# scale-lab/MTLoRA

Measured on AMD Instinct MI355X. Metric: images/sec (train step) Swin-T/448 r=64 4-task, higher is better.
Workload: dtype bf16; 1 GPU; BASELINE configs[1]: Swin-T 448, 4 tasks (semseg,normals,sal,human_parts), r_shared=64 r_task=4 scale4; train step (fwd+loss+bwd+clip+AdamW), dropout .05, drop_path .2; per_gpu_batch=32, global_batch=32, img_size=448, parallelism=dp1, trainable_params=8344634, allreduce_bytes=0

## Files before the change

include/mtlora_hip.h:

```cpp
#ifndef MTLORA_HIP_H
#define MTLORA_HIP_H

#include <stdint.h>

#ifdef __cplusplus
extern "C" {
#endif

#define MTLORA_ABI_VERSION 12
#define MTLORA_MAX_TASKS 8

typedef enum mtlora_dtype {
    MTLORA_F32 = 0,
    MTLORA_BF16 = 1,
    MTLORA_F16 = 2,
    MTLORA_U8 = 3
} mtlora_dtype;

typedef enum mtlora_status {
    MTLORA_OK = 0,
    MTLORA_ERR_DTYPE = -1,
    MTLORA_ERR_SHAPE = -2,
    MTLORA_ERR_ALIGN = -3,
    MTLORA_ERR_NULL = -4,
    MTLORA_ERR_WORKSPACE = -5,
    MTLORA_ERR_HIP = -6,
    MTLORA_ERR_UNSUPPORTED = -7
} mtlora_status;

int mtlora_version(void);
const char* mtlora_error_string(int status);

int mtlora_roll_and_window_partition_forward(const void* image, void* windows, int64_t B, int64_t H, int64_t W,
                                             int64_t C, int shift_size, int window_size, int dtype, void* stream);
int mtlora_roll_and_window_partition_backward(const void* grad_windows, void* grad_image, int64_t B, int64_t H,
                                              int64_t W, int64_t C, int shift_size, int window_size, int dtype,
                                              void* stream);
int mtlora_window_merge_and_roll_forward(const void* windows, void* image, int64_t B, int64_t H, int64_t W,
                                         int64_t C, int shift_size, int window_size, int dtype, void* stream);
int mtlora_window_merge_and_roll_backward(const void* grad_image, void* grad_windows, int64_t B, int64_t H,
                                          int64_t W, int64_t C, int shift_size, int window_size, int dtype,
                                          void* stream);

typedef struct mtlora_linear_desc {
    int64_t M, K, N;
    int32_t dtype;
    int32_t mode;
    int32_t T;
    int32_t r_s;
    int32_t r_t[MTLORA_MAX_TASKS];
    float scale_s;
    float scale_t[MTLORA_MAX_TASKS];
    int32_t has_x_tasks;
    float dropout_p;
    uint64_t seed;
    const uint64_t* seed_offset;
    int32_t bwd_phase;
    int32_t sel_stream;
    int32_t sel_dense;
    int32_t sel_tn;
    int32_t sel_projk;
    int32_t max_cu;
    const void* packed;
    int32_t hid;
    int32_t hid_pad_;
    const void* hid_ptr;
} mtlora_linear_desc;

#define MTLORA_HID_FWD_BASE 1
#define MTLORA_HID_P_GIVEN 2
#define MTLORA_HID_Q_GIVEN 4

int64_t mtlora_linear_ctx_bytes(const mtlora_linear_desc* d);

int64_t mtlora_linear_packed_bytes(const mtlora_linear_desc* d);
int mtlora_linear_pack(const mtlora_linear_desc* d, const float* A_s, const float* B_s, const float* const* A_t,
                       const float* const* B_t, void* packed, int64_t packed_bytes, void* stream);
int64_t mtlora_linear_pack_entry_bytes(void);
int mtlora_linear_pack_entry(const mtlora_linear_desc* d, const float* A_s, const float* B_s, const float* const* A_t,
                             const float* const* B_t, void* packed, int64_t packed_bytes, void* entry_host);
int mtlora_linear_pack_table(const void* table_dev, int n_entries, int dtype, void* stream);
int64_t mtlora_linear_bwd_scratch_bytes(const mtlora_linear_desc* d);

int mtlora_linear_fwd(const mtlora_linear_desc* d, const void* x, const void* const* x_t, const void* W,
                      const float* bias, const float* A_s, const float* B_s, const float* const* A_t,
                      const float* const* B_t, void* y_s, void* const* y_t, void* ctx, int64_t ctx_bytes,
                      void* stream);

int mtlora_linear_bwd(const mtlora_linear_desc* d, const void* x, const void* const* x_t, const void* Wt,
                      const void* dy_s, const void* const* dy_t, const void* ctx, int64_t ctx_bytes, void* dx,
                      void* const* dx_t, float* dA_s, float* dB_s, float* const* dA_t, float* const* dB_t,
                      void* scratch, int64_t scratch_bytes, void* stream);

int mtlora_linear_fwd_gelu(const mtlora_linear_desc* d, const void* x, const void* const* x_t, const void* W,
                           const float* bias, const float* A_s, const float* B_s, const float* const* A_t,
                           const float* const* B_t, void* y_s, void* const* y_t, void* a_s, void* const* a_t, void* ctx,
                           int64_t ctx_bytes, void* stream);

int mtlora_linear_bwd_gelu(const mtlora_linear_desc* d, const void* x, const void* const* x_t, const void* Wt,
                           const void* dy_s, const void* const* dy_t, const void* ctx, int64_t ctx_bytes, void* dx,
                           void* const* dx_t, float* dA_s, float* dB_s, float* const* dA_t, float* const* dB_t,
                           void* scratch, int64_t scratch_bytes, const void* h_s, const void* const* h_t, void* stream);

int mtlora_mlp_hid_supported(const mtlora_linear_desc* d1, const mtlora_linear_desc* d2);
int64_t mtlora_mlp_hid_fwd_scratch_bytes(const mtlora_linear_desc* d1, const mtlora_linear_desc* d2);
int64_t mtlora_mlp_hid_bwd_scratch_bytes(const mtlora_linear_desc* d1, const mtlora_linear_desc* d2);
int mtlora_mlp_hid_proj(const mtlora_linear_desc* d1, const mtlora_linear_desc* d2, const void* h_base, const void* ctx1,
                        void* ctx2, void* scratch, int64_t scratch_bytes, void* stream);
int mtlora_mlp_hid_bwd(const mtlora_linear_desc* d1, const mtlora_linear_desc* d2, const void* h_base, const void* dh_s,
                       const void* ctx1, const void* ctx2, const void* scratch2, void* scratch1, void* g, float* const* dB1_t,
                       float* const* dA2_t, void* part, int64_t part_bytes, void* stream);

int64_t mtlora_gemm_tn_scratch_bytes(int64_t M, int Na, int Nb);
int mtlora_gemm_tn(const void* a, const void* b, float* out, int64_t M, int Na, int Nb, int64_t lda, int64_t ldb,
                   int dtype, void* scratch, int64_t scratch_bytes, void* stream);

typedef struct mtlora_attn_desc {
    int64_t B;
    int32_t H, W;
    int32_t window_size;
    int32_t shift;
    int32_t num_heads;
    int32_t head_dim;
    int32_t image_layout;
    int32_t dtype;
    float scale;
    float mask_value;
} mtlora_attn_desc;

int64_t mtlora_window_attn_bwd_scratch_bytes(const mtlora_attn_desc* d);

int mtlora_window_attn_fwd(const mtlora_attn_desc* d, const void* qkv, const float* bias, const float* mask,
                           const int32_t* mask_ids, void* out, void* stream);
int mtlora_window_attn_bwd(const mtlora_attn_desc* d, const void* qkv, const float* bias, const float* mask,
                           const int32_t* mask_ids, const void* dout, void* dqkv, float* dbias, void* scratch,
                           int64_t scratch_bytes, void* stream);

int mtlora_layernorm_fwd(const void* x, const float* gamma, const float* beta, void* y, float* mean, float* rstd,
                         int64_t M, int64_t C, float eps, int x_dtype, int y_dtype, int merge_h, int merge_w, void* stream);
int64_t mtlora_layernorm_bwd_scratch_bytes(int64_t M, int64_t C, int x_dtype);
int mtlora_layernorm_bwd(const void* dy, const void* x, const float* gamma, const float* mean, const float* rstd,
                         void* dx, float* dgamma, float* dbeta, int64_t M, int64_t C, int x_dtype, int dy_dtype,
                         void* scratch, int64_t scratch_bytes, const void* dx_addend, int merge_h, int merge_w, void* stream);

int mtlora_residual_layernorm_fwd(const void* shortcut, const void* branch, const float* scale, int64_t B, const float* gamma,
                                  const float* beta, void* x_new, void* y, float* mean, float* rstd, int64_t M, int64_t C,
                                  float eps, int x_dtype, int y_dtype, void* stream);
int mtlora_residual_layernorm_bwd(const void* dy, const void* x_new, const float* gamma, const float* mean, const float* rstd,
                                  void* d_shortcut, void* d_branch, float* dgamma, float* dbeta, const float* scale,
                                  int64_t B, int64_t M, int64_t C, int x_dtype, int dy_dtype, void* scratch,
                                  int64_t scratch_bytes, const void* dx_addend, void* stream);

int64_t mtlora_layernorm_multi_bwd_scratch_bytes(int n, int64_t M, int64_t C, int x_dtype);
int mtlora_layernorm_multi_fwd(int n, const void* const* x, const float* gamma, const float* beta, void* const* y,
                               float* const* mean, float* const* rstd, int64_t M, int64_t C, float eps, int x_dtype, int y_dtype,
                               int merge_h, int merge_w, void* stream);
int mtlora_layernorm_multi_bwd(int n, const void* const* dy, const void* const* x, const float* gamma, const float* const* mean,
                               const float* const* rstd, void* const* dx, float* dgamma, float* dbeta, int64_t M, int64_t C,
                               int x_dtype, int dy_dtype, void* scratch, int64_t scratch_bytes, const void* const* dx_addend,
                               int merge_h, int merge_w, void* stream);

int mtlora_residual_layernorm_streams_fwd(int n, const void* const* res, const void* const* branch, const float* scale,
                                          int64_t B, const float* gamma, const float* beta, void* const* x_new, void* const* y,
                                          float* const* mean, float* const* rstd, int64_t M, int64_t C, float eps, int x_dtype,
                                          int y_dtype, int merge_h, int merge_w, void* stream);
int mtlora_residual_layernorm_streams_bwd(int n, const void* const* dy, const void* const* x_new, const float* gamma,
                                          const float* const* mean, const float* const* rstd, void* const* d_res,
                                          void* const* d_branch, float* dgamma, float* dbeta, const float* scale, int64_t B,
                                          int64_t M, int64_t C, int x_dtype, int dy_dtype, void* scratch, int64_t scratch_bytes,
                                          const void* const* dx_addend, int merge_h, int merge_w, void* stream);

int mtlora_residual_layernorm_multi_fwd(int n, const void* shortcut, const void* const* branch, const float* scale, int64_t B,
                                        const float* gamma, const float* beta, void* const* x_new, void* const* y,
                                        float* const* mean, float* const* rstd, int64_t M, int64_t C, float eps, int x_dtype,
                                        int y_dtype, void* stream);
int mtlora_residual_layernorm_multi_bwd(int n, const void* const* dy, const void* const* x_new, const float* gamma,
                                        const float* const* mean, const float* const* rstd, const void* const* dx_addend,
                                        void* d_shortcut, void* const* d_branch, float* dgamma, float* dbeta, const float* scale,
                                        int64_t B, int64_t M, int64_t C, int x_dtype, int dy_dtype, void* scratch,
                                        int64_t scratch_bytes, void* stream);

int64_t mtlora_bn_scratch_bytes(int64_t R, int64_t C, int dtype);
int mtlora_bn_relu_fwd(const void* x, const float* gamma, const float* beta, float* running_mean, float* running_var,
                       float momentum, float eps, int relu, void* y, float* save_mean, float* save_rstd,
                       float* save_scale, float* save_shift, int64_t R, int64_t C, int dtype, void* scratch,
                       int64_t scratch_bytes, void* stream);
int mtlora_bn_relu_bwd(const void* dy, const void* x, const float* save_mean, const float* save_rstd,
                       const float* save_scale, const float* save_shift, int relu, void* dx, float* dgamma, float* dbeta,
                       int64_t R, int64_t C, int dtype, void* scratch, int64_t scratch_bytes, void* stream);

int mtlora_residual_droppath_fwd(int n, const void* const* res, const void* const* y, void* const* out,
                                 const float* scale, int64_t M, int64_t C, int64_t B, int res_dtype, int y_dtype,
                                 void* stream);
int mtlora_residual_droppath_bwd(int n, const void* const* g, void* const* dy, void* dres, const float* scale,
                                 int64_t M, int64_t C, int64_t B, int res_dtype, int y_dtype, void* stream);

int64_t mtlora_upsample_loss_partials(int64_t B, int h, int w, int scale);
int mtlora_upsample_loss(int kind, const void* low, const float* label, const float* stat, void* dlow, float* partials,
                         int64_t B, int h, int w, int C, int scale, int dtype, float ignore_index, void* stream);

int mtlora_upsample_metrics_sizes(int kind, int64_t B, int h, int w, int C, int scale, int64_t* n_int64,
                                  int64_t* n_float_partials);
int mtlora_upsample_metrics(int kind, const void* low, const float* label, const float* stat, int64_t* counts,
                            float* fpartials, int64_t B, int h, int w, int C, int scale, int dtype, float ignore_index,
                            void* stream);

int mtlora_upsample_predict(int kind, const void* low, void* out, int64_t B, int h, int w, int C, int scale, int dtype,
                            int out_dtype, void* stream);

int64_t mtlora_colsum_scratch_bytes(int64_t M, int64_t N);
int mtlora_colsum(const void* x, int64_t M, int64_t N, int dtype, float* out, void* scratch, int64_t scratch_bytes, void* stream);
int64_t mtlora_label_stat_scratch_bytes(int64_t n);
int mtlora_label_stat(const float* label, int64_t n, int kind, float ignore_index, float* out, void* scratch,
                      int64_t scratch_bytes, void* stream);

int mtlora_upsample_cl_fwd(const void* coarse, void* fine, int64_t B, int h, int w, int C, int scale, int64_t ld_fine,
                           int dtype, void* stream);
int mtlora_upsample_cl_bwd(const void* grad_fine, void* grad_coarse, int64_t B, int h, int w, int C, int scale,
                           int64_t ld_fine, int dtype, void* stream);

typedef struct mtlora_block_desc {
    int64_t B;
    int32_t H, W, C, hidden;
    int32_t num_heads, window_size, shift;
    int32_t dtype;
    int32_t x_dtype;
    int32_t has_norm1;
    float eps1, eps2, eps_next;
    float attn_scale, mask_value;
    mtlora_linear_desc lin[4];
} mtlora_block_desc;

typedef struct mtlora_block_params {
    const float *norm1_g, *norm1_b;
    const float *norm2_g, *norm2_b, *next_g, *next_b;
    const void* W[4];
    const void* Wt[4];
    const float* bias[4];
    const float* A[4];
    const float* Bf[4];
    const float* attn_bias;
    const int32_t* mask_ids;
    const float* mask;
    const float *scale1, *scale2;
} mtlora_block_params;

typedef struct mtlora_block_grads {
    void* g_x;
    void* g_normed;
    float *d_norm1_g, *d_norm1_b;
    float *d_norm2_g, *d_norm2_b, *d_next_g, *d_next_b;
    float* dA[4];
    float* dB[4];
    float* dbias;
} mtlora_block_grads;

int64_t mtlora_block_save_bytes(const mtlora_block_desc* d);
int64_t mtlora_block_fwd_tmp_bytes(const mtlora_block_desc* d);
int64_t mtlora_block_bwd_scratch_bytes(const mtlora_block_desc* d);
int mtlora_block_fwd(const mtlora_block_desc* d, const mtlora_block_params* p, const void* x, const void* normed, void* x_out,
                     void* normed_out, void* save, int64_t save_bytes, void* tmp, int64_t tmp_bytes, void* stream);
int mtlora_block_bwd(const mtlora_block_desc* d, const mtlora_block_params* p, const void* x, const void* normed,
                     const void* x_out, const void* g_x_out, const void* g_normed_out, const void* save, int64_t save_bytes,
                     const mtlora_block_grads* g, void* scratch, int64_t scratch_bytes, int phase, void* stream);

#define MTLORA_ADAMW_CHUNK 4096
#define MTLORA_ADAMW_MAX_GROUPS 16
#define MTLORA_ADAMW_CTRL_WORDS 64
// ... 80 lines not shown
```

mtlora_amd/_lib.py:

```python
from __future__ import annotations

import ctypes
import os
from ctypes import POINTER, Structure, c_char_p, c_double, c_float, c_int, c_int32, c_int64, c_uint64, c_void_p

import torch

MAX_TASKS = 8
ABI_VERSION = 12
F32, BF16, F16, U8 = 0, 1, 2, 3
_DT = {torch.float32: F32, torch.bfloat16: BF16, torch.float16: F16}

_HERE = os.path.dirname(os.path.abspath(__file__))
LIB_PATH = os.path.join(_HERE, "csrc", "libmtlora_hip.so")


class LinearDesc(Structure):
    _fields_ = [("M", c_int64), ("K", c_int64), ("N", c_int64), ("dtype", c_int32), ("mode", c_int32),
                ("T", c_int32), ("r_s", c_int32), ("r_t", c_int32 * MAX_TASKS), ("scale_s", c_float),
                ("scale_t", c_float * MAX_TASKS), ("has_x_tasks", c_int32), ("dropout_p", c_float),
                ("seed", c_uint64), ("seed_offset", c_void_p), ("bwd_phase", c_int32),
                ("sel_stream", c_int32), ("sel_dense", c_int32), ("sel_tn", c_int32), ("sel_projk", c_int32),
                ("max_cu", c_int32), ("packed", c_void_p),
                ("hid", c_int32), ("hid_pad_", c_int32), ("hid_ptr", c_void_p)]


HID_FWD_BASE, HID_P_GIVEN, HID_Q_GIVEN = 1, 2, 4


class AttnDesc(Structure):
    _fields_ = [("B", c_int64), ("H", c_int32), ("W", c_int32), ("window_size", c_int32), ("shift", c_int32),
                ("num_heads", c_int32), ("head_dim", c_int32), ("image_layout", c_int32), ("dtype", c_int32),
                ("scale", c_float), ("mask_value", c_float)]


class BlockDesc(Structure):
    _fields_ = [("B", c_int64), ("H", c_int32), ("W", c_int32), ("C", c_int32), ("hidden", c_int32), ("num_heads", c_int32),
                ("window_size", c_int32), ("shift", c_int32), ("dtype", c_int32), ("x_dtype", c_int32), ("has_norm1", c_int32),
                ("eps1", c_float), ("eps2", c_float), ("eps_next", c_float), ("attn_scale", c_float), ("mask_value", c_float),
                ("lin", LinearDesc * 4)]


class BlockParams(Structure):
    _fields_ = [("norm1_g", c_void_p), ("norm1_b", c_void_p), ("norm2_g", c_void_p), ("norm2_b", c_void_p), ("next_g", c_void_p),
                ("next_b", c_void_p), ("W", c_void_p * 4), ("Wt", c_void_p * 4), ("bias", c_void_p * 4), ("A", c_void_p * 4),
                ("Bf", c_void_p * 4), ("attn_bias", c_void_p), ("mask_ids", c_void_p), ("mask", c_void_p), ("scale1", c_void_p),
                ("scale2", c_void_p)]


class BlockGrads(Structure):
    _fields_ = [("g_x", c_void_p), ("g_normed", c_void_p), ("d_norm1_g", c_void_p), ("d_norm1_b", c_void_p), ("d_norm2_g", c_void_p),
                ("d_norm2_b", c_void_p), ("d_next_g", c_void_p), ("d_next_b", c_void_p), ("dA", c_void_p * 4), ("dB", c_void_p * 4),
                ("dbias", c_void_p)]


class AdamwGroup(Structure):
    _fields_ = [("lr", c_double), ("beta1", c_double), ("beta2", c_double), ("eps", c_double), ("weight_decay", c_double)]


class IngestJob(Structure):
    _fields_ = [("src", c_void_p), ("dst", c_void_p), ("kind", c_int32), ("src_dtype", c_int32), ("C", c_int32),
                ("reserved", c_int32)]


class AugmentJob(Structure):
    _fields_ = [("src", c_void_p), ("dst", c_void_p), ("kind", c_int32), ("flags", c_int32)]


INGEST_MAX_JOBS = 8
AUGMENT_IMAGE_CUBIC_U8, AUGMENT_CLASS_NEAREST_U8, AUGMENT_NORMALS_CUBIC_F32, AUGMENT_DEPTH_NEAREST_F32 = 0, 1, 2, 3
AUGMENT_GEOM_BITS, AUGMENT_FLAG_NO_RENORM = 24, 1
INGEST_IMAGE, INGEST_CLASS, INGEST_CLASS_ALLZERO_IGNORE, INGEST_NORMALS, INGEST_DEPTH = 0, 1, 2, 3, 4

ADAMW_CHUNK, ADAMW_MAX_GROUPS, ADAMW_CTRL_WORDS = 4096, 16, 64
ADAMW_GROUPS_DEV_BYTES = 1152
ADAMW_CTRL_MICRO, ADAMW_CTRL_UPDATED = 5, 6
ADAMW_MAX_ACCUM_STEPS = 1 << 24

PROF_KINDS = 24


class ProfSummary(Structure):
    _fields_ = [("count", c_int64 * PROF_KINDS), ("ms", ctypes.c_double * PROF_KINDS),
                ("alg_bytes", ctypes.c_double * PROF_KINDS), ("s8d_bytes", ctypes.c_double * PROF_KINDS),
                ("flops", ctypes.c_double * PROF_KINDS)]


PtrArr = c_void_p * MAX_TASKS
PtrArr9 = c_void_p * (MAX_TASKS + 1)

_SIGS = {
    "mtlora_version": (c_int, []),
    "mtlora_error_string": (c_char_p, [c_int]),
    "mtlora_roll_and_window_partition_forward": (c_int, [c_void_p, c_void_p, c_int64, c_int64, c_int64, c_int64, c_int, c_int, c_int, c_void_p]),
    "mtlora_roll_and_window_partition_backward": (c_int, [c_void_p, c_void_p, c_int64, c_int64, c_int64, c_int64, c_int, c_int, c_int, c_void_p]),
    "mtlora_window_merge_and_roll_forward": (c_int, [c_void_p, c_void_p, c_int64, c_int64, c_int64, c_int64, c_int, c_int, c_int, c_void_p]),
    "mtlora_window_merge_and_roll_backward": (c_int, [c_void_p, c_void_p, c_int64, c_int64, c_int64, c_int64, c_int, c_int, c_int, c_void_p]),
    "mtlora_linear_ctx_bytes": (c_int64, [POINTER(LinearDesc)]),
    "mtlora_linear_bwd_scratch_bytes": (c_int64, [POINTER(LinearDesc)]),
    "mtlora_linear_packed_bytes": (c_int64, [POINTER(LinearDesc)]),
    "mtlora_linear_pack": (c_int, [POINTER(LinearDesc), c_void_p, c_void_p, POINTER(c_void_p), POINTER(c_void_p), c_void_p, c_int64,
                                   c_void_p]),
    "mtlora_linear_pack_entry_bytes": (c_int64, []),
    "mtlora_linear_pack_entry": (c_int, [POINTER(LinearDesc), c_void_p, c_void_p, POINTER(c_void_p), POINTER(c_void_p), c_void_p, c_int64,
                                         c_void_p]),
    "mtlora_linear_pack_table": (c_int, [c_void_p, c_int, c_int, c_void_p]),
    "mtlora_linear_fwd": (c_int, [POINTER(LinearDesc), c_void_p, POINTER(c_void_p), c_void_p, c_void_p, c_void_p, c_void_p,
                                  POINTER(c_void_p), POINTER(c_void_p), c_void_p, POINTER(c_void_p), c_void_p, c_int64,
                                  c_void_p]),
    "mtlora_linear_bwd": (c_int, [POINTER(LinearDesc), c_void_p, POINTER(c_void_p), c_void_p, c_void_p, POINTER(c_void_p),
                                  c_void_p, c_int64, c_void_p, POINTER(c_void_p), c_void_p, c_void_p, POINTER(c_void_p),
                                  POINTER(c_void_p), c_void_p, c_int64, c_void_p]),
    "mtlora_gemm_tn_scratch_bytes": (c_int64, [c_int64, c_int, c_int]),
    "mtlora_gemm_tn": (c_int, [c_void_p, c_void_p, c_void_p, c_int64, c_int, c_int, c_int64, c_int64, c_int, c_void_p, c_int64,
                               c_void_p]),
    "mtlora_linear_fwd_gelu": (c_int, [POINTER(LinearDesc), c_void_p, POINTER(c_void_p), c_void_p, c_void_p, c_void_p, c_void_p,
                                       POINTER(c_void_p), POINTER(c_void_p), c_void_p, POINTER(c_void_p), c_void_p,
                                       POINTER(c_void_p), c_void_p, c_int64, c_void_p]),
    "mtlora_linear_bwd_gelu": (c_int, [POINTER(LinearDesc), c_void_p, POINTER(c_void_p), c_void_p, c_void_p, POINTER(c_void_p),
                                       c_void_p, c_int64, c_void_p, POINTER(c_void_p), c_void_p, c_void_p, POINTER(c_void_p),
                                       POINTER(c_void_p), c_void_p, c_int64, c_void_p, POINTER(c_void_p), c_void_p]),
    "mtlora_mlp_hid_supported": (c_int, [POINTER(LinearDesc), POINTER(LinearDesc)]),
    "mtlora_mlp_hid_bwd_scratch_bytes": (c_int64, [POINTER(LinearDesc), POINTER(LinearDesc)]),
    "mtlora_mlp_hid_fwd_scratch_bytes": (c_int64, [POINTER(LinearDesc), POINTER(LinearDesc)]),
    "mtlora_mlp_hid_proj": (c_int, [POINTER(LinearDesc), POINTER(LinearDesc), c_void_p, c_void_p, c_void_p, c_void_p, c_int64, c_void_p]),
    "mtlora_mlp_hid_bwd": (c_int, [POINTER(LinearDesc), POINTER(LinearDesc), c_void_p, c_void_p, c_void_p, c_void_p, c_void_p, c_void_p,
                                   c_void_p, POINTER(c_void_p), POINTER(c_void_p), c_void_p, c_int64, c_void_p]),
    "mtlora_window_attn_bwd_scratch_bytes": (c_int64, [POINTER(AttnDesc)]),
    "mtlora_window_attn_fwd": (c_int, [POINTER(AttnDesc), c_void_p, c_void_p, c_void_p, c_void_p, c_void_p, c_void_p]),
    "mtlora_window_attn_bwd": (c_int, [POINTER(AttnDesc), c_void_p, c_void_p, c_void_p, c_void_p, c_void_p, c_void_p,
                                       c_void_p, c_void_p, c_int64, c_void_p]),
    "mtlora_layernorm_fwd": (c_int, [c_void_p, c_void_p, c_void_p, c_void_p, c_void_p, c_void_p, c_int64, c_int64, c_float,
                                     c_int, c_int, c_int, c_int, c_void_p]),
    "mtlora_layernorm_bwd_scratch_bytes": (c_int64, [c_int64, c_int64, c_int]),
    "mtlora_residual_layernorm_fwd": (c_int, [c_void_p, c_void_p, c_void_p, c_int64, c_void_p, c_void_p, c_void_p, c_void_p,
                                              c_void_p, c_void_p, c_int64, c_int64, c_float, c_int, c_int, c_void_p]),
    "mtlora_layernorm_multi_bwd_scratch_bytes": (c_int64, [c_int, c_int64, c_int64, c_int]),
    "mtlora_layernorm_multi_fwd": (c_int, [c_int, POINTER(c_void_p), c_void_p, c_void_p, POINTER(c_void_p), POINTER(c_void_p),
                                           POINTER(c_void_p), c_int64, c_int64, c_float, c_int, c_int, c_int, c_int, c_void_p]),
    "mtlora_layernorm_multi_bwd": (c_int, [c_int, POINTER(c_void_p), POINTER(c_void_p), c_void_p, POINTER(c_void_p),
                                           POINTER(c_void_p), POINTER(c_void_p), c_void_p, c_void_p, c_int64, c_int64, c_int,
                                           c_int, c_void_p, c_int64, POINTER(c_void_p), c_int, c_int, c_void_p]),
    "mtlora_residual_layernorm_streams_fwd": (c_int, [c_int, POINTER(c_void_p), POINTER(c_void_p), c_void_p, c_int64, c_void_p,
                                                      c_void_p, POINTER(c_void_p), POINTER(c_void_p), POINTER(c_void_p),
                                                      POINTER(c_void_p), c_int64, c_int64, c_float, c_int, c_int, c_int, c_int,
                                                      c_void_p]),
    "mtlora_residual_layernorm_streams_bwd": (c_int, [c_int, POINTER(c_void_p), POINTER(c_void_p), c_void_p, POINTER(c_void_p),
                                                      POINTER(c_void_p), POINTER(c_void_p), POINTER(c_void_p), c_void_p, c_void_p,
                                                      c_void_p, c_int64, c_int64, c_int64, c_int, c_int, c_void_p, c_int64,
                                                      POINTER(c_void_p), c_int, c_int, c_void_p]),
    "mtlora_residual_layernorm_multi_fwd": (c_int, [c_int, c_void_p, POINTER(c_void_p), c_void_p, c_int64, c_void_p, c_void_p,
                                                    POINTER(c_void_p), POINTER(c_void_p), POINTER(c_void_p), POINTER(c_void_p),
                                                    c_int64, c_int64, c_float, c_int, c_int, c_void_p]),
    "mtlora_residual_layernorm_multi_bwd": (c_int, [c_int, POINTER(c_void_p), POINTER(c_void_p), c_void_p, POINTER(c_void_p),
                                                    POINTER(c_void_p), POINTER(c_void_p), c_void_p, POINTER(c_void_p), c_void_p,
                                                    c_void_p, c_void_p, c_int64, c_int64, c_int64, c_int, c_int, c_void_p, c_int64,
                                                    c_void_p]),
    "mtlora_residual_layernorm_bwd": (c_int, [c_void_p, c_void_p, c_void_p, c_void_p, c_void_p, c_void_p, c_void_p, c_void_p,
                                              c_void_p, c_void_p, c_int64, c_int64, c_int64, c_int, c_int, c_void_p, c_int64,
                                              c_void_p, c_void_p]),
    "mtlora_layernorm_bwd": (c_int, [c_void_p, c_void_p, c_void_p, c_void_p, c_void_p, c_void_p, c_void_p, c_void_p,
                                     c_int64, c_int64, c_int, c_int, c_void_p, c_int64, c_void_p, c_int, c_int, c_void_p]),
    "mtlora_bn_scratch_bytes": (c_int64, [c_int64, c_int64, c_int]),
    "mtlora_bn_relu_fwd": (c_int, [c_void_p, c_void_p, c_void_p, c_void_p, c_void_p, c_float, c_float, c_int, c_void_p,
                                   c_void_p, c_void_p, c_void_p, c_void_p, c_int64, c_int64, c_int, c_void_p, c_int64,
                                   c_void_p]),
    "mtlora_bn_relu_bwd": (c_int, [c_void_p, c_void_p, c_void_p, c_void_p, c_void_p, c_void_p, c_int, c_void_p, c_void_p,
                                   c_void_p, c_int64, c_int64, c_int, c_void_p, c_int64, c_void_p]),
    "mtlora_residual_droppath_fwd": (c_int, [c_int, POINTER(c_void_p), POINTER(c_void_p), POINTER(c_void_p), c_void_p,
                                             c_int64, c_int64, c_int64, c_int, c_int, c_void_p]),
    "mtlora_residual_droppath_bwd": (c_int, [c_int, POINTER(c_void_p), POINTER(c_void_p), c_void_p, c_void_p, c_int64,
                                             c_int64, c_int64, c_int, c_int, c_void_p]),
    "mtlora_upsample_loss_partials": (c_int64, [c_int64, c_int, c_int, c_int]),
    "mtlora_colsum_scratch_bytes": (c_int64, [c_int64, c_int64]),
    "mtlora_colsum": (c_int, [c_void_p, c_int64, c_int64, c_int, c_void_p, c_void_p, c_int64, c_void_p]),
    "mtlora_label_stat_scratch_bytes": (c_int64, [c_int64]),
    "mtlora_label_stat": (c_int, [c_void_p, c_int64, c_int, c_float, c_void_p, c_void_p, c_int64, c_void_p]),
    "mtlora_upsample_loss": (c_int, [c_int, c_void_p, c_void_p, c_void_p, c_void_p, c_void_p, c_int64, c_int, c_int, c_int,
                                     c_int, c_int, ctypes.c_float, c_void_p]),
    "mtlora_upsample_metrics_sizes": (c_int, [c_int, c_int64, c_int, c_int, c_int, c_int, POINTER(c_int64), POINTER(c_int64)]),
    "mtlora_upsample_metrics": (c_int, [c_int, c_void_p, c_void_p, c_void_p, c_void_p, c_void_p, c_int64, c_int, c_int, c_int,
                                        c_int, c_int, ctypes.c_float, c_void_p]),
    "mtlora_upsample_predict": (c_int, [c_int, c_void_p, c_void_p, c_int64, c_int, c_int, c_int, c_int, c_int, c_int, c_void_p]),
    "mtlora_upsample_cl_fwd": (c_int, [c_void_p, c_void_p, c_int64, c_int, c_int, c_int, c_int, c_int64, c_int, c_void_p]),
    "mtlora_upsample_cl_bwd": (c_int, [c_void_p, c_void_p, c_int64, c_int, c_int, c_int, c_int, c_int64, c_int, c_void_p]),
    "mtlora_block_save_bytes": (c_int64, [POINTER(BlockDesc)]),
    "mtlora_block_fwd_tmp_bytes": (c_int64, [POINTER(BlockDesc)]),
    "mtlora_block_bwd_scratch_bytes": (c_int64, [POINTER(BlockDesc)]),
    "mtlora_block_fwd": (c_int, [POINTER(BlockDesc), POINTER(BlockParams), c_void_p, c_void_p, c_void_p, c_void_p, c_void_p, c_int64,
                                 c_void_p, c_int64, c_void_p]),
    "mtlora_block_bwd": (c_int, [POINTER(BlockDesc), POINTER(BlockParams), c_void_p, c_void_p, c_void_p, c_void_p, c_void_p, c_void_p,
                                 c_int64, POINTER(BlockGrads), c_void_p, c_int64, c_int, c_void_p]),
    "mtlora_adamw_sizes": (c_int, [c_int64, POINTER(c_int64), POINTER(c_int64), POINTER(c_int64), POINTER(c_int64)]),
    "mtlora_adamw_table": (c_int, [c_int64, POINTER(c_int64), POINTER(c_int32), POINTER(c_void_p), POINTER(c_void_p), POINTER(c_void_p),
                                   c_void_p, c_int64]),
    "mtlora_adamw_update": (c_int, [c_void_p, c_void_p, c_int64, c_int64, POINTER(AdamwGroup), c_int, c_float, c_void_p, c_void_p,
                                    c_void_p, c_void_p, c_float, c_float, c_int, c_void_p, c_int64, c_void_p]),
    "mtlora_adamw_update_dev": (c_int, [c_void_p, c_void_p, c_int64, c_int64, c_void_p, c_int, c_float, c_void_p, c_void_p,
                                        c_void_p, c_void_p, c_double, c_double, c_int, c_void_p, c_int64, c_void_p]),
    "mtlora_adamw_accum_layout": (c_int, [c_int64, POINTER(c_int64), POINTER(c_int64), POINTER(c_int64)]),
    "mtlora_adamw_accum_update_dev": (c_int, [c_void_p, c_void_p, c_int64, c_int64, c_void_p, c_int, c_float, c_void_p, c_void_p,
                                              c_void_p, c_void_p, c_double, c_double, c_int, c_void_p, c_int64, c_void_p, c_void_p,
                                              c_int, c_void_p]),
    "mtlora_ingest_scratch_bytes": (c_int64, [c_int, c_int64]),
    "mtlora_ingest_batch": (c_int, [POINTER(IngestJob), c_int, c_int64, c_int32, c_int32, c_void_p, c_void_p, c_void_p, c_int64,
                                    c_void_p]),
    "mtlora_augment_batch": (c_int, [POINTER(AugmentJob), c_int, c_int64, c_int32, c_int32, c_int32, c_int32, c_void_p, c_void_p,
                                     c_void_p, c_void_p, c_void_p, c_void_p]),
    "mtlora_selftest_layouts": (c_int, [c_void_p, c_void_p]),
    "mtlora_prof_begin": (c_int, [c_int]),
    "mtlora_prof_end": (c_int, [POINTER(ProfSummary)]),
    "mtlora_prof_kind_name": (c_char_p, [c_int]),
}
EXPORTS = tuple(_SIGS)

_lib = None


def lib() -> ctypes.CDLL:
    global _lib
    if _lib is None:
        if not os.path.exists(LIB_PATH):
            raise RuntimeError(
                f"mtlora_amd: {LIB_PATH} not found. Build it with `python -m mtlora_amd.csrc.build` "
                "(or __graft_entry__.build()). There is no eager/CPU fallback for the MTLoRA hot path.")
        L = ctypes.CDLL(LIB_PATH)
        for name, (res, args) in _SIGS.items():
            fn = getattr(L, name)
            fn.restype, fn.argtypes = res, args
        v = L.mtlora_version()
        if v != ABI_VERSION:
            raise RuntimeError(f"mtlora_amd: libmtlora_hip.so ABI {v} != binding ABI {ABI_VERSION}; rebuild")
        _lib = L
    return _lib


def check(status: int, what: str) -> None:
    if status != 0:
        msg = lib().mtlora_error_string(status).decode()
        raise RuntimeError(f"mtlora_amd: {what} failed: {msg} (status {status})")


def dtype_code(t: torch.Tensor, allow_f16: bool = True) -> int:
    code = _DT.get(t.dtype)
    if code is None or (code == F16 and not allow_f16):
        raise RuntimeError(f"mtlora_amd: unsupported dtype {t.dtype} (fp32, bf16 and fp16 are supported)")
    return code


def require_gpu(*tensors: torch.Tensor) -> None:
    cur = None
    for t in tensors:
        if t is None:
            continue
        if not t.is_cuda:
            raise RuntimeError("mtlora_amd: tensors must live on a ROCm GPU (MI355X); the HIP path has no CPU fallback")
        if cur is None:
            cur = torch._C._cuda_getDevice()
        if t.device.index != cur:
            raise RuntimeError(f"mtlora_amd: tensor on cuda:{t.device.index} but the current device is cuda:{cur}; the HIP "
                               "path launches on the current device's stream -- call torch.cuda.set_device(tensor.device) first")


def ptr(t) -> c_void_p:
    return c_void_p(0 if t is None else t.data_ptr())


_NO_PTRS = None
# ... 24 lines not shown
```

mtlora_amd/csrc/build.py:

```python
import os
import subprocess
import sys
from concurrent.futures import ThreadPoolExecutor

HERE = os.path.dirname(os.path.abspath(__file__))
SOURCES = ["window_process.hip", "linear.hip", "attention.hip", "glue.hip", "layernorm.hip", "loss.hip", "metrics.hip", "predict.hip", "upsample.hip", "reduce.hip", "selftest.hip", "block.hip", "hid.hip", "optim.hip", "ingest.hip", "augment.hip"]
LIB = os.path.join(HERE, "libmtlora_hip.so")
FLAGS = ["--offload-arch=gfx950", "-O3", "-std=c++17", "-fPIC", "-Wno-unused-value", "-Wno-unused-result"]


def _hipcc():
    for c in (os.environ.get("HIPCC"), "/opt/rocm/bin/hipcc", "hipcc"):
        if c and (os.path.isabs(c) and os.path.exists(c) or not os.path.isabs(c)):
            return c
    return "hipcc"


def _stale(target, deps):
    if not os.path.exists(target):
        return True
    t = os.path.getmtime(target)
    return any(os.path.getmtime(d) > t for d in deps)


def build(force=False, verbose=True):
    hdrs = [os.path.join(HERE, f) for f in sorted(os.listdir(HERE)) if f.endswith(".h")]
    hdrs.append(os.path.join(HERE, "..", "..", "include", "mtlora_hip.h"))
    objs, jobs = [], []
    for src in SOURCES:
        s = os.path.join(HERE, src)
        o = os.path.join(HERE, src.replace(".hip", ".o"))
        objs.append(o)
        if force or _stale(o, [s] + hdrs):
            jobs.append([_hipcc()] + FLAGS + ["-c", s, "-o", o])
    if jobs:
        def run(cmd):
            if verbose:
                print(" ".join(cmd), flush=True)
            subprocess.run(cmd, check=True, cwd=HERE)
        with ThreadPoolExecutor(max_workers=4) as ex:
            list(ex.map(run, jobs))
    if jobs or force or _stale(LIB, objs):
        cmd = [_hipcc(), "--offload-arch=gfx950", "-shared", "-fPIC", "-o", LIB] + objs
        if verbose:
            print(" ".join(cmd), flush=True)
        subprocess.run(cmd, check=True, cwd=HERE)
    return LIB


if __name__ == "__main__":
    print(build(force="--force" in sys.argv))
```

mtlora_amd/csrc/common.h:

```cpp
#pragma once
#include <hip/hip_runtime.h>
#include <stdint.h>

#include "../../include/mtlora_hip.h"

typedef __bf16 bf16;
typedef __attribute__((ext_vector_type(8))) __bf16 bf16x8;
typedef __attribute__((ext_vector_type(4))) __bf16 bf16x4;
typedef _Float16 f16;
typedef __attribute__((ext_vector_type(8))) _Float16 f16x8;
typedef __attribute__((ext_vector_type(4))) _Float16 f16x4;
typedef __attribute__((ext_vector_type(16))) float f32x16;
typedef __attribute__((ext_vector_type(4))) float f32x4;
typedef __attribute__((ext_vector_type(4))) uint32_t u32x4;
typedef __attribute__((ext_vector_type(2))) uint32_t u32x2;
typedef __attribute__((ext_vector_type(4))) short s16x4;

#define MTL_WAVE 64

#define MTL_CHECK_LAUNCH()                                   \
    do {                                                     \
        hipError_t e__ = hipGetLastError();                  \
        if (e__ != hipSuccess) return MTLORA_ERR_HIP;        \
    } while (0)
// ... 168 lines not shown
}
template <typename T, bool CVT>
__device__ __forceinline__ u32x4 mtl_gelu_pk4(const u32x4& v) {
    u32x4 o;
#pragma unroll
    for (int q2 = 0; q2 < 4; q2 += 2) {
        f32x2 h[2], er[2];
#pragma unroll
        for (int q = 0; q < 2; ++q) h[q] = f32x2{mtl_lo2<T>(v[q2 + q]), mtl_hi2<T>(v[q2 + q])};
        mtl_erf2n<2>(h, er);
#pragma unroll
        for (int q = 0; q < 2; ++q) {
            const f32x2 a = h[q] * (0.5f + 0.5f * er[q]);
            o[q2 + q] = CVT ? mtl_pk2<T>(a.x, a.y) : mtl_pack2<T>(a.x, a.y);
        }
    }
    return o;
}
template <typename T, bool CVT>
__device__ __forceinline__ u32x4 mtl_gelu_gate_pk4(const u32x4& g, const u32x4& hv) {
    u32x4 o;
#pragma unroll
    for (int q2 = 0; q2 < 4; q2 += 2) {
        f32x2 h[2], er[2];
#pragma unroll
        for (int q = 0; q < 2; ++q) h[q] = f32x2{mtl_lo2<T>(hv[q2 + q]), mtl_hi2<T>(hv[q2 + q])};
        mtl_erf2n<2>(h, er);
#pragma unroll
        for (int q = 0; q < 2; ++q) {
            const f32x2 cdf = 0.5f + 0.5f * er[q];
            const f32x2 qq = h[q] * h[q];
            const f32x2 e = {__builtin_amdgcn_exp2f(qq.x * -0.72134752044448170f), __builtin_amdgcn_exp2f(qq.y * -0.72134752044448170f)};
            const f32x2 d = (cdf + h[q] * e * 0.39894228040143268f) * f32x2{mtl_lo2<T>(g[q2 + q]), mtl_hi2<T>(g[q2 + q])};
            o[q2 + q] = CVT ? mtl_pk2<T>(d.x, d.y) : mtl_pack2<T>(d.x, d.y);
        }
    }
    return o;
}

template <typename T>
struct VOps;
template <>
struct VOps<bf16> {
    static constexpr int N = 8;
    static __device__ __forceinline__ void unpack(const u32x4& v, float (&f)[8]) {
#pragma unroll
        for (int w = 0; w < 4; ++w) {
            f[2 * w] = __builtin_bit_cast(float, v[w] << 16);
            f[2 * w + 1] = __builtin_bit_cast(float, v[w] & 0xFFFF0000u);
        }
    }
    static __device__ __forceinline__ u32x4 pack(const float (&f)[8]) {
        return u32x4{mtl_pack_bf16(f[0], f[1]), mtl_pack_bf16(f[2], f[3]), mtl_pack_bf16(f[4], f[5]),
                     mtl_pack_bf16(f[6], f[7])};
    }
    static __device__ __forceinline__ void drop(u32x4& v, const DropoutCfg& c, uint32_t rowhash, uint32_t k) {
#pragma unroll
        for (int w = 0; w < 4; ++w) {
            const uint32_t h = mtl_dropout_pairbits(c, rowhash, k + 2 * w);
            uint32_t keep = 0u;
            if ((h & 0xFFFFu) >= c.thr16) keep |= 0x0000FFFFu;
            if ((h >> 16) >= c.thr16) keep |= 0xFFFF0000u;
            v[w] &= keep;
        }
    }
};
template <>
struct VOps<f16> {
    static constexpr int N = 8;
    static __device__ __forceinline__ void unpack(const u32x4& v, float (&f)[8]) {
#pragma unroll
        for (int w = 0; w < 4; ++w) {
            f[2 * w] = mtl_lo2<f16>(v[w]);
            f[2 * w + 1] = mtl_hi2<f16>(v[w]);
        }
    }
    static __device__ __forceinline__ u32x4 pack(const float (&f)[8]) {
        return u32x4{mtl_pack_f16(f[0], f[1]), mtl_pack_f16(f[2], f[3]), mtl_pack_f16(f[4], f[5]), mtl_pack_f16(f[6], f[7])};
    }
    static __device__ __forceinline__ void drop(u32x4& v, const DropoutCfg& c, uint32_t rowhash, uint32_t k) {
        VOps<bf16>::drop(v, c, rowhash, k);
    }
};
template <>
struct VOps<float> {
    static constexpr int N = 4;
    static __device__ __forceinline__ void unpack(const u32x4& v, float (&f)[8]) {
#pragma unroll
        for (int w = 0; w < 4; ++w) f[w] = __builtin_bit_cast(float, v[w]);
    }
    static __device__ __forceinline__ u32x4 pack(const float (&f)[8]) {
        return u32x4{__builtin_bit_cast(uint32_t, f[0]), __builtin_bit_cast(uint32_t, f[1]),
                     __builtin_bit_cast(uint32_t, f[2]), __builtin_bit_cast(uint32_t, f[3])};
    }
    static __device__ __forceinline__ void drop(u32x4& v, const DropoutCfg& c, uint32_t rowhash, uint32_t k) {
#pragma unroll
        for (int p = 0; p < 2; ++p) {
            const uint32_t h = mtl_dropout_pairbits(c, rowhash, k + 2 * p);
            if ((h & 0xFFFFu) < c.thr16) v[2 * p] = 0u;
            if ((h >> 16) < c.thr16) v[2 * p + 1] = 0u;
        }
    }
};

template <typename T>
struct Frag {
    u32x4 v[2];
};

__device__ __forceinline__ void mtl_mma(const Frag<bf16>& a, const Frag<bf16>& b, f32x16& c) {
    c = __builtin_amdgcn_mfma_f32_32x32x16_bf16(__builtin_bit_cast(bf16x8, a.v[0]), __builtin_bit_cast(bf16x8, b.v[0]),
                                                c, 0, 0, 0);
    c = __builtin_amdgcn_mfma_f32_32x32x16_bf16(__builtin_bit_cast(bf16x8, a.v[1]), __builtin_bit_cast(bf16x8, b.v[1]),
                                                c, 0, 0, 0);
}
__device__ __forceinline__ void mtl_mma(const Frag<f16>& a, const Frag<f16>& b, f32x16& c) {
    c = __builtin_amdgcn_mfma_f32_32x32x16_f16(__builtin_bit_cast(f16x8, a.v[0]), __builtin_bit_cast(f16x8, b.v[0]), c, 0, 0, 0);
    c = __builtin_amdgcn_mfma_f32_32x32x16_f16(__builtin_bit_cast(f16x8, a.v[1]), __builtin_bit_cast(f16x8, b.v[1]), c, 0, 0, 0);
}
__device__ __forceinline__ void mtl_mma(const Frag<float>& a, const Frag<float>& b, f32x16& c) {
#pragma unroll
    for (int h = 0; h < 2; ++h) {
        f32x4 av = __builtin_bit_cast(f32x4, a.v[h]);
        f32x4 bv = __builtin_bit_cast(f32x4, b.v[h]);
#pragma unroll
        for (int e = 0; e < 4; ++e) c = __builtin_amdgcn_mfma_f32_32x32x2f32(av[e], bv[e], c, 0, 0, 0);
    }
}

__device__ __forceinline__ int mtl_d_row(int lane, int reg) { return (reg & 3) + 8 * (reg >> 2) + 4 * (lane >> 5); }
__device__ __forceinline__ int mtl_d_col(int lane) { return lane & 31; }

enum MtlProfKind {
    PK_NT_FWD_MAIN = 0,
    PK_NT_FWD_P = 1,
    PK_NT_BWD_Q = 2,
    PK_NT_BWD_DX = 3,
    PK_TN = 4,
    PK_ATTN_FWD = 5,
    PK_ATTN_BWD = 6,
    PK_PACK = 7,
    PK_REDUCE = 8,
    PK_WINDOW = 9,
    PK_LN_FWD = 10,
    PK_LN_BWD = 11,
    PK_RESIDUAL = 13,
    PK_BN = 12,
    PK_LOSS = 14,
    PK_SUM = 15,
    PK_UPSAMPLE = 16,
    PK_NT_PLAIN_FWD = 17,
    PK_NT_PLAIN_DX = 18,
    PK_TN_PLAIN = 19,
    PK_COUNT = 24
};
int mtl_prof_start(int kind, double alg_bytes, hipStream_t s, double s8d_bytes = 0.0, double flops = 0.0);
void mtl_prof_tag(const char* fmt, ...);
void mtl_prof_stop(int idx, hipStream_t s);
struct MtlProfScope {
    int idx;
    hipStream_t s;
    MtlProfScope(int kind, double bytes, hipStream_t st, double s8d = 0.0, double flops = 0.0)
        : idx(mtl_prof_start(kind, bytes, st, s8d, flops)), s(st) {}
    ~MtlProfScope() {
        if (idx >= 0) mtl_prof_stop(idx, s);
    }
};
```

mtlora_amd/csrc/internal.h:

```cpp
#pragma once
#include <stdint.h>

#include "../../include/mtlora_hip.h"

#define MTL_INTERNAL extern "C" __attribute__((visibility("hidden")))

MTL_INTERNAL int mtli_layernorm_bwd(const void* dy, const void* x, const float* gamma, const float* mean, const float* rstd, void* dx,
                                    float* dgamma, float* dbeta, int64_t M, int64_t C, int x_dtype, int dy_dtype, void* scratch,
                                    int64_t scratch_bytes, const void* dx_addend, int phase, void* stream);
MTL_INTERNAL int mtli_residual_layernorm_bwd(const void* dy, const void* x_new, const float* gamma, const float* mean, const float* rstd,
                                             void* d_shortcut, void* d_branch, float* dgamma, float* dbeta, const float* scale,
                                             int64_t B, int64_t M, int64_t C, int x_dtype, int dy_dtype, void* scratch,
                                             int64_t scratch_bytes, const void* dx_addend, int phase, void* stream);

struct HidLaunch;
struct HidParams;
struct HidRedParams;
MTL_INTERNAL void mtli_hid_launch(const HidLaunch* L, const HidParams* q, void* stream);
MTL_INTERNAL void mtli_hid_rows_finish(int dtype, const float* rowpart, int n_chunk, int64_t M, int nt, const float* alpha, const int* off,
                                       void* out, int ldo, void* stream);
MTL_INTERNAL void mtli_hid_reduce(const HidRedParams* r, int64_t per, void* stream);
```

mtlora_amd/csrc/linear.hip:

```cpp
#include <string.h>
#include <algorithm>
#include <atomic>
#include <type_traits>

#include "common.h"
#include "internal.h"
#include "hid_params.h"
#include "nt.h"
#include "stream.h"
#include "dense.h"
#include "pq.h"
#include "tn.h"

namespace {

static Segs make_segs(const mtlora_linear_desc* d) {
    Segs s;
    s.n = 1 + d->T;
    int off = 0;
    for (int o = 0; o < s.n; ++o) {
        int r = (o == 0) ? d->r_s : d->r_t[o - 1];
        s.r[o] = r;
        s.rp[o] = (int)mtl_round_up(r, 8);
        s.off[o] = off;
// ... 1878 lines not shown
    if (((uintptr_t)table_dev & 7u) != 0) return MTLORA_ERR_ALIGN;
    hipStream_t s = (hipStream_t)stream;
    const PackEntry* tb = reinterpret_cast<const PackEntry*>(table_dev);
    MtlProfScope prof(PK_PACK, 0.0, s);
    const dim3 g(256, (unsigned)n_entries);
    if (dtype == MTLORA_F32)
        hipLaunchKernelGGL(k_pack_table<float>, g, dim3(256), 0, s, tb);
    else if (dtype == MTLORA_F16)
        hipLaunchKernelGGL(k_pack_table<f16>, g, dim3(256), 0, s, tb);
    else
        hipLaunchKernelGGL(k_pack_table<bf16>, g, dim3(256), 0, s, tb);
    MTL_CHECK_LAUNCH();
    return MTLORA_OK;
}

static int linear_fwd_entry(const mtlora_linear_desc* d, const void* x, const void* const* x_t, const void* W,
                            const float* bias, const float* A_s, const float* B_s, const float* const* A_t,
                            const float* const* B_t, void* y_s, void* const* y_t, void* a_s, void* const* a_t, void* ctx,
                            int64_t ctx_bytes, void* stream) {
    int st = check_desc(d);
    if (st != MTLORA_OK) return st;
    if (!x || !W || !y_s) return MTLORA_ERR_NULL;
    if (d->r_s > 0 && !d->packed && (!A_s || !B_s)) return MTLORA_ERR_NULL;
    if (misaligned(x) || misaligned(W) || misaligned(y_s) || misaligned(bias) || misaligned(d->packed)) return MTLORA_ERR_ALIGN;
    const bool hid_base = (d->hid & MTLORA_HID_FWD_BASE) != 0, hid_p = (d->hid & MTLORA_HID_P_GIVEN) != 0;
    if (hid_base && (!d->hid_ptr || d->T < 1 || !d->has_x_tasks || d->mode != 0)) return MTLORA_ERR_NULL;
    if (hid_base && misaligned(d->hid_ptr)) return MTLORA_ERR_ALIGN;
    if (hid_p && (d->T < 1 || !d->has_x_tasks || d->mode != 0)) return MTLORA_ERR_UNSUPPORTED;
    for (int t = 0; t < d->T; ++t) {
        if (!hid_base && (!y_t || !y_t[t])) return MTLORA_ERR_NULL;
        if (!d->packed && (!A_t || !B_t || !A_t[t] || !B_t[t])) return MTLORA_ERR_NULL;
        if (!hid_base && misaligned(y_t[t])) return MTLORA_ERR_ALIGN;
        if (d->has_x_tasks && !hid_p && (!x_t || !x_t[t])) return MTLORA_ERR_NULL;
        if (d->has_x_tasks && !hid_p && misaligned(x_t[t])) return MTLORA_ERR_ALIGN;
    }
    const Segs sg = make_segs(d);
    if (sg.R > 0) {
        if (!ctx) return MTLORA_ERR_NULL;
        if (misaligned(ctx)) return MTLORA_ERR_ALIGN;
        if (ctx_bytes < ctx_layout(d, sg).total) return MTLORA_ERR_WORKSPACE;
    }
    if (d->M == 0) return MTLORA_OK;
    hipStream_t s = (hipStream_t)stream;
    if (d->dtype == MTLORA_F32)
        st = fwd_impl<float>(d, x, x_t, W, bias, A_s, B_s, A_t, B_t, y_s, y_t, ctx, s, a_s, a_t);
    else if (d->dtype == MTLORA_F16)
        st = fwd_impl<f16>(d, x, x_t, W, bias, A_s, B_s, A_t, B_t, y_s, y_t, ctx, s, a_s, a_t);
    else
        st = fwd_impl<bf16>(d, x, x_t, W, bias, A_s, B_s, A_t, B_t, y_s, y_t, ctx, s, a_s, a_t);
    if (st != MTLORA_OK) return st;
    MTL_CHECK_LAUNCH();
    return MTLORA_OK;
}

int mtlora_linear_fwd(const mtlora_linear_desc* d, const void* x, const void* const* x_t, const void* W,
                      const float* bias, const float* A_s, const float* B_s, const float* const* A_t,
                      const float* const* B_t, void* y_s, void* const* y_t, void* ctx, int64_t ctx_bytes,
                      void* stream) {
    return linear_fwd_entry(d, x, x_t, W, bias, A_s, B_s, A_t, B_t, y_s, y_t, nullptr, nullptr, ctx, ctx_bytes, stream);
}

int mtlora_linear_fwd_gelu(const mtlora_linear_desc* d, const void* x, const void* const* x_t, const void* W,
                           const float* bias, const float* A_s, const float* B_s, const float* const* A_t,
                           const float* const* B_t, void* y_s, void* const* y_t, void* a_s, void* const* a_t, void* ctx,
                           int64_t ctx_bytes, void* stream) {
    if (!a_s || !d) return MTLORA_ERR_NULL;
    if (misaligned(a_s)) return MTLORA_ERR_ALIGN;
    for (int t = 0; t < d->T && !(d->hid & MTLORA_HID_FWD_BASE); ++t) {
        if (!a_t || !a_t[t]) return MTLORA_ERR_NULL;
        if (misaligned(a_t[t])) return MTLORA_ERR_ALIGN;
    }
    return linear_fwd_entry(d, x, x_t, W, bias, A_s, B_s, A_t, B_t, y_s, y_t, a_s, a_t, ctx, ctx_bytes, stream);
}

static int linear_bwd_entry(const mtlora_linear_desc* d, const void* x, const void* const* x_t, const void* Wt,
                            const void* dy_s, const void* const* dy_t, const void* ctx, int64_t ctx_bytes, void* dx,
                            void* const* dx_t, float* dA_s, float* dB_s, float* const* dA_t, float* const* dB_t,
                            void* scratch, int64_t scratch_bytes, const void* gate_s, const void* const* gate_t,
                            void* stream) {
    int st = check_desc(d);
    if (st != MTLORA_OK) return st;
    if (!x || !Wt) return MTLORA_ERR_NULL;
    if (misaligned(x) || misaligned(Wt) || misaligned(dx) || misaligned(dy_s)) return MTLORA_ERR_ALIGN;
    const Segs sg = make_segs(d);
    if (sg.R > 0) {
        if (!ctx || !scratch) return MTLORA_ERR_NULL;
        if (misaligned(ctx) || misaligned(scratch)) return MTLORA_ERR_ALIGN;
        if (ctx_bytes < ctx_layout(d, sg).total) return MTLORA_ERR_WORKSPACE;
        if (scratch_bytes < bwd_scratch(d, sg).total) return MTLORA_ERR_WORKSPACE;
    }
    if ((d->hid & MTLORA_HID_Q_GIVEN) && (d->T < 1 || !d->has_x_tasks || d->mode != 0 || misaligned(d->hid_ptr))) return MTLORA_ERR_UNSUPPORTED;
    for (int t = 0; t < d->T; ++t) {
        if (d->has_x_tasks && dA_t && dA_t[t] && (!x_t || !x_t[t])) return MTLORA_ERR_NULL;
        if (d->has_x_tasks && x_t && misaligned(x_t[t])) return MTLORA_ERR_ALIGN;
        if (dy_t && misaligned(dy_t[t])) return MTLORA_ERR_ALIGN;
        if (dx_t && misaligned(dx_t[t])) return MTLORA_ERR_ALIGN;
    }
    if (d->M == 0) return MTLORA_OK;
    hipStream_t s = (hipStream_t)stream;
    if (d->dtype == MTLORA_F32)
        st = bwd_impl<float>(d, x, x_t, Wt, dy_s, dy_t, ctx, dx, dx_t, dA_s, dB_s, dA_t, dB_t, scratch, s, gate_s, gate_t);
    else if (d->dtype == MTLORA_F16)
        st = bwd_impl<f16>(d, x, x_t, Wt, dy_s, dy_t, ctx, dx, dx_t, dA_s, dB_s, dA_t, dB_t, scratch, s, gate_s, gate_t);
    else
        st = bwd_impl<bf16>(d, x, x_t, Wt, dy_s, dy_t, ctx, dx, dx_t, dA_s, dB_s, dA_t, dB_t, scratch, s, gate_s, gate_t);
    if (st != MTLORA_OK) return st;
    MTL_CHECK_LAUNCH();
    return MTLORA_OK;
}

int mtlora_linear_bwd(const mtlora_linear_desc* d, const void* x, const void* const* x_t, const void* Wt,
                      const void* dy_s, const void* const* dy_t, const void* ctx, int64_t ctx_bytes, void* dx,
                      void* const* dx_t, float* dA_s, float* dB_s, float* const* dA_t, float* const* dB_t,
                      void* scratch, int64_t scratch_bytes, void* stream) {
    return linear_bwd_entry(d, x, x_t, Wt, dy_s, dy_t, ctx, ctx_bytes, dx, dx_t, dA_s, dB_s, dA_t, dB_t, scratch, scratch_bytes,
                            nullptr, nullptr, stream);
}

int mtlora_linear_bwd_gelu(const mtlora_linear_desc* d, const void* x, const void* const* x_t, const void* Wt,
                           const void* dy_s, const void* const* dy_t, const void* ctx, int64_t ctx_bytes, void* dx,
                           void* const* dx_t, float* dA_s, float* dB_s, float* const* dA_t, float* const* dB_t,
                           void* scratch, int64_t scratch_bytes, const void* h_s, const void* const* h_t, void* stream) {
    if (!h_s || !dx) return MTLORA_ERR_NULL;
    if (misaligned(h_s)) return MTLORA_ERR_ALIGN;
    for (int t = 0; t < d->T && d->has_x_tasks; ++t) {
        if (dx_t && dx_t[t] && (!h_t || !h_t[t])) return MTLORA_ERR_NULL;
        if (h_t && misaligned(h_t[t])) return MTLORA_ERR_ALIGN;
    }
    return linear_bwd_entry(d, x, x_t, Wt, dy_s, dy_t, ctx, ctx_bytes, dx, dx_t, dA_s, dB_s, dA_t, dB_t, scratch, scratch_bytes,
                            h_s, h_t, stream);
}

static int tn_plan(int64_t M, int Na, int Nb, int& tiles_a, int& tiles_b, int& nsplit, int64_t& rps) {
    tiles_a = (int)mtl_ceil_div(Na, TN_A);
    tiles_b = (int)mtl_ceil_div(Nb, TN_B);
    const int64_t tiles = (int64_t)tiles_a * tiles_b;
    nsplit = (int)(TN_TARGET_CTAS / (tiles > 0 ? tiles : 1));
    const int64_t max_by_rows = mtl_ceil_div(M, 256);
    if (nsplit > max_by_rows) nsplit = (int)max_by_rows;
    if (nsplit > 256) nsplit = 256;
    if (nsplit < 1) nsplit = 1;
    rps = mtl_round_up(mtl_ceil_div(M > 0 ? M : 1, nsplit), 64);
    return MTLORA_OK;
}

int64_t mtlora_gemm_tn_scratch_bytes(int64_t M, int Na, int Nb) {
    if (M < 0 || Na <= 0 || Nb <= 0) return -1;
    int ta, tb, ns;
    int64_t rps;
    tn_plan(M, Na, Nb, ta, tb, ns, rps);
    return (int64_t)ta * tb * ns * TN_TILE * 4 + 256;
}

int mtlora_gemm_tn(const void* a, const void* b, float* out, int64_t M, int Na, int Nb, int64_t lda, int64_t ldb,
                   int dtype, void* scratch, int64_t scratch_bytes, void* stream) {
    if (dtype != MTLORA_F32 && dtype != MTLORA_BF16 && dtype != MTLORA_F16) return MTLORA_ERR_DTYPE;
    const int vec = dtype == MTLORA_F32 ? 4 : 8;
    if (M < 0 || M >= ((int64_t)1 << 31) || Na <= 0 || Nb <= 0 || lda < Na || ldb < Nb) return MTLORA_ERR_SHAPE;
    if (Na % vec || Nb % vec || lda % vec || ldb % vec) return MTLORA_ERR_ALIGN;
    if (Na > 1024) return MTLORA_ERR_UNSUPPORTED;
    if (!out || !scratch || (M > 0 && (!a || !b))) return MTLORA_ERR_NULL;
    if (misaligned(a) || misaligned(b) || misaligned(scratch) || ((uintptr_t)out & 3u)) return MTLORA_ERR_ALIGN;
    if (scratch_bytes < mtlora_gemm_tn_scratch_bytes(M, Na, Nb) - 256) return MTLORA_ERR_WORKSPACE;
    hipStream_t s = (hipStream_t)stream;
    if (M == 0) {
        mtl_zero_async(out, (size_t)Na * Nb * 4, s);
        return MTLORA_OK;
    }
    TnParams tp = {};
    tp.M = M;
    int ta, tb;
    tn_plan(M, Na, Nb, ta, tb, tp.nsplit, tp.rows_per_split);
    tp.drop = mtl_make_dropout(0.f, 0, nullptr);
    tp.n_prob = 1;
    TnProblem& p = tp.p[0];
    p.A = a;
    p.B = b;
    p.lda = lda;
    p.ldb = ldb;
    p.a0 = 0;
    p.Na = Na;
    p.b0 = 0;
    p.Nb = Nb;
    p.b_mask = 0;
    p.tiles_a = ta;
    p.tiles_b = tb;
    p.part = reinterpret_cast<float*>(scratch);
    p.out = out;
    p.out_a = Na;
    p.out_b = Nb;
    p.ldo = Nb;
    p.transpose = 0;
    const int es = mtl_elem_size(dtype);
    {
        mtl_prof_tag("M%lld Na%d Nb%d", (long long)M, Na, Nb);
        MtlProfScope prof(PK_TN_PLAIN, (double)es * M * ((double)ta * Nb + Na), s, 0.0, 2.0 * M * (double)Na * Nb);
        if (dtype == MTLORA_F32)
            hipLaunchKernelGGL(k_tn<float>, dim3((unsigned)tp.nsplit, (unsigned)(ta * tb), 1), dim3(256), 0, s, tp);
        else if (dtype == MTLORA_F16)
            hipLaunchKernelGGL(k_tn<f16>, dim3((unsigned)tp.nsplit, (unsigned)(ta * tb), 1), dim3(256), 0, s, tp);
        else
            hipLaunchKernelGGL(k_tn<bf16>, dim3((unsigned)tp.nsplit, (unsigned)(ta * tb), 1), dim3(256), 0, s, tp);
    }
    MtlProfScope prof(PK_REDUCE, 0.0, s);
    hipLaunchKernelGGL(k_tn_reduce, dim3(TN_TILE / 1024, (unsigned)(ta * tb), 1), dim3(256 * TN_RG), 0, s, tp);
    MTL_CHECK_LAUNCH();
    return MTLORA_OK;
}
}
```

mtlora_amd/csrc/reduce.hip:

```cpp
#include "common.h"

namespace {

constexpr int RD_MAXBLK = 1024;

template <typename T>
__global__ __launch_bounds__(256) void k_colsum_part(const T* x, int64_t M, int N, float* part) {
    constexpr int VE = ET<T>::VEC;
    __shared__ float sm[256][VE + 1];
    const int nvec = N / VE;
    const int tid = threadIdx.x;
    for (int v0 = 0; v0 < nvec; v0 += 256) {
        const int cv = nvec - v0 < 256 ? nvec - v0 : 256;
        const int rps = 256 / cv;
        const int r = tid / cv, v = tid - r * cv;
        float acc[VE];
#pragma unroll
        for (int e = 0; e < VE; ++e) acc[e] = 0.f;
        if (r < rps) {
            for (int64_t m = (int64_t)blockIdx.x * rps + r; m < M; m += (int64_t)gridDim.x * rps) {
                const Vec16<T> q = mtl_ld16<T>(x + m * N + (int64_t)(v0 + v) * VE);
#pragma unroll
                for (int e = 0; e < VE; ++e) acc[e] += mtl_to_f32(q.e[e]);
            }
        }
#pragma unroll
        for (int e = 0; e < VE; ++e) sm[tid][e] = (r < rps) ? acc[e] : 0.f;
        __syncthreads();
        if (tid < cv) {
            float t[VE];
#pragma unroll
            for (int e = 0; e < VE; ++e) t[e] = 0.f;
            for (int rr = 0; rr < rps; ++rr)
#pragma unroll
                for (int e = 0; e < VE; ++e) t[e] += sm[rr * cv + tid][e];
#pragma unroll
            for (int e = 0; e < VE; ++e) part[(int64_t)blockIdx.x * N + (int64_t)(v0 + tid) * VE + e] = t[e];
        }
        __syncthreads();
    }
}

constexpr int RD_RW = 16;
__global__ __launch_bounds__(64 * RD_RW) void k_colsum_combine(const float* part, float* out, int nblk, int N, float scale) {
    __shared__ float sm[RD_RW][64];
    const int lane = threadIdx.x & 63, wave = threadIdx.x >> 6;
    const int c = blockIdx.x * 64 + lane;
    float a0 = 0.f, a1 = 0.f, a2 = 0.f, a3 = 0.f;
    if (c < N) {
        int b = wave;
        for (; b + 3 * RD_RW < nblk; b += 4 * RD_RW) {
            a0 += part[(int64_t)b * N + c];
            a1 += part[(int64_t)(b + RD_RW) * N + c];
            a2 += part[(int64_t)(b + 2 * RD_RW) * N + c];
            a3 += part[(int64_t)(b + 3 * RD_RW) * N + c];
        }
        for (; b < nblk; b += RD_RW) a0 += part[(int64_t)b * N + c];
    }
    sm[wave][lane] = (a0 + a1) + (a2 + a3);
    __syncthreads();
    if (wave == 0 && c < N) {
        float t = 0.f;
#pragma unroll
        for (int w = 0; w < RD_RW; ++w) t += sm[w][lane];
        out[c] = t * scale;
    }
}

__global__ __launch_bounds__(256) void k_label_stat_part(const float* lab, int64_t n, int kind, float ignore, float* part) {
    __shared__ float sm[256];
    float c = 0.f;
    const int64_t nv = n >> 2;
    for (int64_t i = (int64_t)blockIdx.x * 256 + threadIdx.x; i < nv; i += (int64_t)gridDim.x * 256) {
        const f32x4 v = *reinterpret_cast<const f32x4*>(lab + i * 4);
#pragma unroll
        for (int e = 0; e < 4; ++e) c += kind == 0 ? (v[e] != ignore ? 1.f : 0.f) : (v[e] >= 0.5f ? 0.f : 1.f);
    }
    if (blockIdx.x == 0 && threadIdx.x < (int)(n & 3)) {
        const float v = lab[(nv << 2) + threadIdx.x];
        c += kind == 0 ? (v != ignore ? 1.f : 0.f) : (v >= 0.5f ? 0.f : 1.f);
    }
    sm[threadIdx.x] = c;
    __syncthreads();
    for (int s = 128; s > 0; s >>= 1) {
        if (threadIdx.x < s) sm[threadIdx.x] += sm[threadIdx.x + s];
        __syncthreads();
    }
    if (threadIdx.x == 0) part[blockIdx.x] = sm[0];
}

__global__ __launch_bounds__(256) void k_label_stat_combine(const float* part, float* out, int nblk, double scale) {
    __shared__ double sm[256];
    double t = 0.0;
    for (int b = threadIdx.x; b < nblk; b += 256) t += (double)part[b];
    sm[threadIdx.x] = t;
    __syncthreads();
    for (int s = 128; s > 0; s >>= 1) {
        if (threadIdx.x < s) sm[threadIdx.x] += sm[threadIdx.x + s];
        __syncthreads();
    }
    if (threadIdx.x == 0) out[0] = (float)(sm[0] * scale);
}

int rd_blocks(int64_t work_items) {
    int64_t g = mtl_ceil_div(work_items, 256 * 8);
    if (g > RD_MAXBLK) g = RD_MAXBLK;
    return (int)(g < 1 ? 1 : g);
}

}

extern "C" {

int64_t mtlora_colsum_scratch_bytes(int64_t M, int64_t N) {
    if (M < 0 || N <= 0) return -1;
    return (int64_t)RD_MAXBLK * N * 4 + 256;
}

int mtlora_colsum(const void* x, int64_t M, int64_t N, int dtype, float* out, void* scratch, int64_t scratch_bytes, void* stream) {
    if (dtype != MTLORA_F32 && dtype != MTLORA_BF16) return MTLORA_ERR_DTYPE;
    const int ve = dtype == MTLORA_F32 ? 4 : 8;
    if (M < 0 || N <= 0 || N % ve || N > (1 << 20)) return MTLORA_ERR_SHAPE;
    if (!x || !out || !scratch) return MTLORA_ERR_NULL;
    if (((uintptr_t)x | (uintptr_t)scratch) & 15u) return MTLORA_ERR_ALIGN;
    if (scratch_bytes < mtlora_colsum_scratch_bytes(M, N)) return MTLORA_ERR_WORKSPACE;
    hipStream_t s = (hipStream_t)stream;
    const int nvec = (int)(N / ve);
    const int rps = nvec >= 256 ? 1 : 256 / nvec;
    int64_t g = mtl_ceil_div(M, (int64_t)rps * 8);
    if (g > RD_MAXBLK) g = RD_MAXBLK;
    if (g < 1) g = 1;
    float* part = reinterpret_cast<float*>(scratch);
    if (dtype == MTLORA_F32)
        hipLaunchKernelGGL(k_colsum_part<float>, dim3((unsigned)g), dim3(256), 0, s, reinterpret_cast<const float*>(x), M, (int)N, part);
    else
        hipLaunchKernelGGL(k_colsum_part<bf16>, dim3((unsigned)g), dim3(256), 0, s, reinterpret_cast<const bf16*>(x), M, (int)N, part);
    hipLaunchKernelGGL(k_colsum_combine, dim3((unsigned)mtl_ceil_div(N, 64)), dim3(64 * RD_RW), 0, s, (const float*)part, out, (int)g,
                       (int)N, 1.f);
    MTL_CHECK_LAUNCH();
    return MTLORA_OK;
}

int64_t mtlora_label_stat_scratch_bytes(int64_t n) {
    if (n < 0) return -1;
    return (int64_t)RD_MAXBLK * 4 + 256;
}

int mtlora_label_stat(const float* label, int64_t n, int kind, float ignore_index, float* out, void* scratch,
                      int64_t scratch_bytes, void* stream) {
    if (kind != 0 && kind != 1) return MTLORA_ERR_UNSUPPORTED;
    if (n <= 0) return MTLORA_ERR_SHAPE;
    if (!label || !out || !scratch) return MTLORA_ERR_NULL;
    if ((uintptr_t)label & 15u) return MTLORA_ERR_ALIGN;
    if (scratch_bytes < mtlora_label_stat_scratch_bytes(n)) return MTLORA_ERR_WORKSPACE;
    hipStream_t s = (hipStream_t)stream;
    const int g = rd_blocks(n / 4 + 1);
    float* part = reinterpret_cast<float*>(scratch);
    hipLaunchKernelGGL(k_label_stat_part, dim3((unsigned)g), dim3(256), 0, s, label, n, kind, ignore_index, part);
    hipLaunchKernelGGL(k_label_stat_combine, dim3(1), dim3(256), 0, s, (const float*)part, out, g, kind == 0 ? 1.0 : 1.0 / (double)n);
    MTL_CHECK_LAUNCH();
    return MTLORA_OK;
}

}
```

mtlora_amd/csrc/selftest.hip:

```cpp
#include "common.h"
#include <cstdarg>
#include <cstdio>
#include <cstring>

namespace {
__global__ __launch_bounds__(64) void k_selftest(int32_t* out) {
    __shared__ __attribute__((aligned(16))) short lds[1024];
    const int l = threadIdx.x, h = l >> 5, i = l & 31;
    {
        Frag<bf16> a, b;
        a.v[0] = a.v[1] = b.v[0] = b.v[1] = u32x4{0u, 0u, 0u, 0u};
        if (h == 0) {
            bf16 x = (bf16)(float)(i + 1);
            uint32_t bits = (uint32_t)__builtin_bit_cast(uint16_t, x);
            a.v[0][0] = bits;
            b.v[0][0] = bits;
        }
        f32x16 c;
        for (int r = 0; r < 16; ++r) c[r] = 0.f;
        mtl_mma(a, b, c);
        for (int r = 0; r < 16; ++r) out[l * 16 + r] = (int32_t)c[r];
    }
    {
        Frag<float> a, b;
        a.v[0] = a.v[1] = b.v[0] = b.v[1] = u32x4{0u, 0u, 0u, 0u};
        if (h == 0) {
            a.v[0][0] = __builtin_bit_cast(uint32_t, (float)(i + 1));
            b.v[0][0] = a.v[0][0];
        }
        f32x16 c;
        for (int r = 0; r < 16; ++r) c[r] = 0.f;
        mtl_mma(a, b, c);
        for (int r = 0; r < 16; ++r) out[1024 + l * 16 + r] = (int32_t)c[r];
    }
    for (int x = l; x < 1024; x += 64) lds[x] = (short)x;
    __syncthreads();
    {
        s16x4 v = __builtin_amdgcn_ds_read_tr16_b64_v4i16((__attribute__((address_space(3))) s16x4*)(lds + l * 4));
        for (int e = 0; e < 4; ++e) out[2048 + l * 4 + e] = (int32_t)v[e];
    }
    {
        const int g = l >> 4, ig = l & 15;
        const int row = 2 * g + (ig >> 2);
        const int col = 16 * (g & 1) + 4 * (ig & 3);
        s16x4 v = __builtin_amdgcn_ds_read_tr16_b64_v4i16(
            (__attribute__((address_space(3))) s16x4*)(lds + row * 72 + col));
        for (int e = 0; e < 4; ++e) out[2304 + l * 4 + e] = (int32_t)v[e];
    }
}
}

extern "C" int mtlora_selftest_layouts(int32_t* out, void* stream) {
    if (!out) return MTLORA_ERR_NULL;
    hipLaunchKernelGGL(k_selftest, dim3(1), dim3(64), 0, (hipStream_t)stream, out);
    MTL_CHECK_LAUNCH();
    return MTLORA_OK;
}

#include <atomic>
#include <mutex>
#include <vector>
namespace {
struct ProfRec {
    int kind;
    double bytes, s8d, flops;
    hipEvent_t a, b;
    char tag[56];
};
thread_local char g_next_tag[56] = {0};
std::atomic<int> g_prof_on{0};
std::mutex g_prof_mu;
std::vector<ProfRec> g_prof;
size_t g_prof_cap = 0;
}

int mtl_prof_start(int kind, double alg_bytes, hipStream_t s, double s8d_bytes, double flops) {
    if (!g_prof_on.load(std::memory_order_relaxed)) return -1;
    std::lock_guard<std::mutex> lk(g_prof_mu);
    if (g_prof.size() >= g_prof_cap) return -1;
    ProfRec r;
    r.kind = kind;
    r.bytes = alg_bytes;
    r.s8d = s8d_bytes;
    r.flops = flops;
    memcpy(r.tag, g_next_tag, sizeof(r.tag));
    g_next_tag[0] = 0;
    if (hipEventCreate(&r.a) != hipSuccess) return -1;
    if (hipEventCreate(&r.b) != hipSuccess) {
        (void)hipEventDestroy(r.a);
        return -1;
    }
    (void)hipEventRecord(r.a, s);
    g_prof.push_back(r);
    return (int)g_prof.size() - 1;
}
void mtl_prof_tag(const char* fmt, ...) {
    if (!g_prof_on.load(std::memory_order_relaxed)) return;
    va_list ap;
    va_start(ap, fmt);
    vsnprintf(g_next_tag, sizeof(g_next_tag), fmt, ap);
    va_end(ap);
}
void mtl_prof_stop(int idx, hipStream_t s) {
    std::lock_guard<std::mutex> lk(g_prof_mu);
    if (idx >= 0 && (size_t)idx < g_prof.size()) (void)hipEventRecord(g_prof[idx].b, s);
}

extern "C" int mtlora_prof_begin(int max_records) {
    std::lock_guard<std::mutex> lk(g_prof_mu);
    for (auto& r : g_prof) {
        (void)hipEventDestroy(r.a);
        (void)hipEventDestroy(r.b);
    }
    g_prof.clear();
    g_prof_cap = max_records > 0 ? (size_t)max_records : 0;
    g_prof.reserve(g_prof_cap);
    g_prof_on.store(1);
    return MTLORA_OK;
}

extern "C" int mtlora_prof_end(mtlora_prof_summary* out) {
    g_prof_on.store(0);
    std::lock_guard<std::mutex> lk(g_prof_mu);
    if (out) {
        for (int k = 0; k < MTLORA_PROF_KINDS; ++k) {
            out->count[k] = 0;
            out->ms[k] = 0.0;
            out->alg_bytes[k] = 0.0;
            out->s8d_bytes[k] = 0.0;
            out->flops[k] = 0.0;
        }
    }
    int st = MTLORA_OK;
    const char* dump = getenv("MTLORA_PROF_DUMP");
    FILE* df = dump && dump[0] ? fopen(dump, "w") : nullptr;
    for (auto& r : g_prof) {
        float ms = 0.f;
        if (hipEventSynchronize(r.b) != hipSuccess || hipEventElapsedTime(&ms, r.a, r.b) != hipSuccess) st = MTLORA_ERR_HIP;
        if (df) fprintf(df, "%s,%.0f,%.0f,%.0f,%.4f,%s\n", mtlora_prof_kind_name(r.kind), r.bytes, r.s8d, r.flops, ms, r.tag);
        if (out && r.kind >= 0 && r.kind < MTLORA_PROF_KINDS) {
            out->count[r.kind] += 1;
            out->ms[r.kind] += ms;
            out->alg_bytes[r.kind] += r.bytes;
            out->s8d_bytes[r.kind] += r.s8d;
            out->flops[r.kind] += r.flops;
        }
        (void)hipEventDestroy(r.a);
        (void)hipEventDestroy(r.b);
    }
    if (df) fclose(df);
    g_prof.clear();
    return st;
}

extern "C" const char* mtlora_prof_kind_name(int kind) {
    switch (kind) {
        case PK_NT_FWD_MAIN: return "k_nt:fwd_outputs";
        case PK_NT_FWD_P: return "k_nt:fwd_lowrank_P";
        case PK_NT_BWD_Q: return "k_nt:bwd_lowrank_Q";
        case PK_NT_BWD_DX: return "k_nt:bwd_dX";
        case PK_TN: return "k_tn:dA_dB";
        case PK_ATTN_FWD: return "k_attn_fwd";
        case PK_ATTN_BWD: return "k_attn_bwd";
        case PK_PACK: return "k_pack";
        case PK_REDUCE: return "k_tn_reduce";
        case PK_WINDOW: return "k_window_process";
        case PK_LN_FWD: return "k_ln_fwd";
        case PK_LN_BWD: return "k_ln_bwd";
        case PK_BN: return "k_bn";
        case PK_RESIDUAL: return "k_residual";
        case PK_LOSS: return "k_up_loss";
        case PK_SUM: return "k_sum";
        case PK_UPSAMPLE: return "k_upsample";
        case PK_NT_PLAIN_FWD: return "k_nt:plain_fwd";
        case PK_NT_PLAIN_DX: return "k_nt:plain_dX";
        case PK_TN_PLAIN: return "k_tn:plain_dW";
        default: return "";
    }
}
```

mtlora_amd/functional.py:

```python
from __future__ import annotations

import ctypes
import os
from dataclasses import dataclass, field
from typing import List, Optional, Sequence, Tuple

import torch

from . import _lib as L

_seed_counter = 0


_seed_offset: Optional[torch.Tensor] = None


def set_seed_offset(t: Optional[torch.Tensor]) -> None:
    global _seed_offset
    if t is not None and not (t.is_cuda and t.dtype == torch.int64 and t.numel() == 1):
        raise RuntimeError("mtlora_amd: the seed offset must be a CUDA int64 tensor with one element")
    _seed_offset = t


_factor_stream: Optional["torch.cuda.Stream"] = None
# ... 1309 lines not shown
        stat = label_stat(lab, 0, ignore_index)
    elif kind == "saliency":
        stat = torch.cat([label_stat(lab, 1, ignore_index), saliency_thresholds(lab.device)])
    elif kind == "edge":
        stat = torch.full((1,), float(pos_weight), dtype=torch.float32, device=lab.device)
    else:
        raise RuntimeError(f"mtlora_amd: unknown fused metrics kind {kind!r}")
    ni, nfp = upsample_metrics_sizes(kind, B, h, w, C, scale)
    if counts is None:
        counts = torch.zeros(max(ni, 1), dtype=torch.int64, device=lo.device)
    elif counts.dtype != torch.int64 or counts.numel() < ni or not counts.is_contiguous() or counts.device != lo.device:
        raise RuntimeError(f"mtlora_amd: counts must be a contiguous int64 tensor of at least {ni} elements on {lo.device}")
    nq = METRIC_FLOATS[kind]
    part = torch.empty(max(nfp, nq), dtype=torch.float32, device=lo.device)
    st = L.lib().mtlora_upsample_metrics(METRIC_KINDS[kind], L.ptr(lo), L.ptr(lab), L.ptr(stat), L.ptr(counts), L.ptr(part), B, h,
                                         w, C, int(scale), L.dtype_code(lo), float(ignore_index), L.stream_ptr())
    L.check(st, "mtlora_upsample_metrics")
    if nfp == 0:
        return counts, torch.zeros(nq, dtype=torch.float64, device=lo.device)
    return counts, part[:nfp].view(nq, nfp // nq).sum(1, dtype=torch.float64)


PREDICT_KINDS = {"argmax": 0, "normals": 1, "sigmoid": 2, "identity": 3}
_PREDICT_OUT = {"argmax": (torch.uint8,), "normals": (torch.float32, torch.uint8), "sigmoid": (torch.float32, torch.uint8),
                "identity": (torch.float32,)}


@torch.no_grad()
def upsample_predict(kind: str, low, scale: int, out_dtype=None, out=None):
    if kind not in PREDICT_KINDS:
        raise RuntimeError(f"mtlora_amd: unknown fused prediction kind {kind!r}")
    L.require_gpu(low, out)
    B, h, w, C = low.shape
    H, W = h * int(scale), w * int(scale)
    if out_dtype is None:
        out_dtype = _PREDICT_OUT[kind][0] if out is None else out.dtype
    if out_dtype not in _PREDICT_OUT[kind]:
        raise RuntimeError(f"mtlora_amd: fused prediction kind {kind!r} writes {_PREDICT_OUT[kind]}, not {out_dtype}")
    shape = {"argmax": (B, H, W), "normals": (B, H, W, C), "sigmoid": (B, H, W), "identity": (B, H, W, 1)}[kind]
    lo = low.detach().contiguous()
    if lo.dtype not in (torch.float32, torch.bfloat16, torch.float16):
        lo = lo.float()
    if out is None:
        out = torch.empty(shape, dtype=out_dtype, device=lo.device)
    elif tuple(out.shape) != shape or out.dtype != out_dtype or not out.is_contiguous() or out.device != lo.device:
        raise RuntimeError(f"mtlora_amd: out must be a contiguous {out_dtype} tensor of shape {shape} on {lo.device}")
    st = L.lib().mtlora_upsample_predict(PREDICT_KINDS[kind], L.ptr(lo), L.ptr(out), B, h, w, C, int(scale), L.dtype_code(lo),
                                         L.U8 if out_dtype == torch.uint8 else L.F32, L.stream_ptr())
    L.check(st, "mtlora_upsample_predict")
    return out


INGEST_KINDS = {"image": L.INGEST_IMAGE, "class": L.INGEST_CLASS, "class_allzero_ignore": L.INGEST_CLASS_ALLZERO_IGNORE,
                "normals": L.INGEST_NORMALS, "depth": L.INGEST_DEPTH}
_INGEST_SRC = {torch.uint8: L.U8, torch.float32: L.F32, torch.float16: L.F16}


def ingest_batch(jobs, flip=None, lut=None):
    jobs = list(jobs)
    srcs = [s for _, s in jobs]
    L.require_gpu(*srcs, flip, lut)
    if not jobs:
        raise RuntimeError("mtlora_amd: ingest_batch needs at least one job")
    B, H, W = srcs[0].shape[:3]
    arr = (L.IngestJob * max(len(jobs), 1))()
    outs = []
    for i, (kind, src) in enumerate(jobs):
        if kind not in INGEST_KINDS:
            raise RuntimeError(f"mtlora_amd: unknown ingest kind {kind!r}")
        C = src.shape[3] if src.dim() == 4 else 1
        if src.dim() not in (3, 4) or tuple(src.shape[:3]) != (B, H, W) or not src.is_contiguous():
            raise RuntimeError(f"mtlora_amd: ingest job {i} ({kind}) must be a contiguous (B, H, W[, C]) tensor with "
                               f"B, H, W = {(B, H, W)}, got {tuple(src.shape)}")
        if src.dtype not in _INGEST_SRC:
            raise RuntimeError(f"mtlora_amd: unsupported dtype {src.dtype} for an ingest source (uint8, fp32 and fp16 are supported)")
        out = torch.empty((B, C, H, W), dtype=torch.float32, device=src.device)
        outs.append(out)
        arr[i].src, arr[i].dst, arr[i].kind, arr[i].src_dtype, arr[i].C = src.data_ptr(), out.data_ptr(), INGEST_KINDS[kind], \
            _INGEST_SRC[src.dtype], C
    if flip is not None and (flip.dtype != torch.uint8 or tuple(flip.shape) != (B,) or not flip.is_contiguous()):
        raise RuntimeError(f"mtlora_amd: flip must be a contiguous uint8 tensor of shape ({B},)")
    if lut is not None and (lut.dtype != torch.float32 or tuple(lut.shape) != (3, 256) or not lut.is_contiguous()):
        raise RuntimeError("mtlora_amd: lut must be a contiguous fp32 tensor of shape (3, 256)")
    scratch, nbytes = None, 0
    if any(kind == "class_allzero_ignore" for kind, _ in jobs):
        nbytes = int(L.lib().mtlora_ingest_scratch_bytes(len(jobs), B))
        if nbytes > 0:
            scratch = torch.empty(nbytes, dtype=torch.uint8, device=srcs[0].device)
    st = L.lib().mtlora_ingest_batch(arr, len(jobs), B, H, W, L.ptr(flip), L.ptr(lut), L.ptr(scratch), nbytes, L.stream_ptr())
    L.check(st, "mtlora_ingest_batch")
    return outs


AUGMENT_KINDS = {"image_cubic_u8": L.AUGMENT_IMAGE_CUBIC_U8, "class_nearest_u8": L.AUGMENT_CLASS_NEAREST_U8,
                 "normals_cubic_f32": L.AUGMENT_NORMALS_CUBIC_F32, "depth_nearest_f32": L.AUGMENT_DEPTH_NEAREST_F32}
_AUGMENT_FORM = {"image_cubic_u8": (torch.uint8, 3), "class_nearest_u8": (torch.uint8, 1), "normals_cubic_f32": (torch.float32, 3),
                 "depth_nearest_f32": (torch.float32, 1)}


def augment_batch(jobs, size, coef, side, out_size, cubic_q15=None, cubic_f32=None, renormalize=True):
    jobs = list(jobs)
    srcs = [s for _, s in jobs]
    L.require_gpu(*srcs, size, coef, side, cubic_q15, cubic_f32)
    if not jobs:
        raise RuntimeError("mtlora_amd: augment_batch needs at least one job")
    B, Hc, Wc = srcs[0].shape[:3]
    Ho, Wo = int(out_size[0]), int(out_size[1])
    for name, t, dt, shape in (("size", size, torch.int32, (B, 2)), ("coef", coef, torch.int64, (B, 6)), ("side", side, torch.float32, (B, 3)),
                               ("cubic_q15", cubic_q15, torch.int32, (32, 4)), ("cubic_f32", cubic_f32, torch.float32, (32, 4))):
        if t is not None and (t.dtype != dt or tuple(t.shape) != shape or not t.is_contiguous()):
            raise RuntimeError(f"mtlora_amd: {name} must be a contiguous {dt} tensor of shape {shape}, got {t.dtype} {tuple(t.shape)}")
    arr = (L.AugmentJob * max(len(jobs), 1))()
    outs = []
    for i, (kind, src) in enumerate(jobs):
        if kind not in AUGMENT_KINDS:
            raise RuntimeError(f"mtlora_amd: unknown augment kind {kind!r}")
        dt, C = _AUGMENT_FORM[kind]
        want = (B, Hc, Wc, 3) if C == 3 else (B, Hc, Wc)
        if src.dtype != dt or tuple(src.shape) != want or not src.is_contiguous():
            raise RuntimeError(f"mtlora_amd: augment job {i} ({kind}) must be a contiguous {dt} tensor of shape {want}, got "
                               f"{src.dtype} {tuple(src.shape)}")
        out = torch.empty((B, Ho, Wo, 3) if C == 3 else (B, Ho, Wo), dtype=dt, device=src.device)
        outs.append(out)
        arr[i].src, arr[i].dst, arr[i].kind = src.data_ptr(), out.data_ptr(), AUGMENT_KINDS[kind]
        arr[i].flags = 0 if renormalize else L.AUGMENT_FLAG_NO_RENORM
    st = L.lib().mtlora_augment_batch(arr, len(jobs), B, Hc, Wc, Ho, Wo, L.ptr(size), L.ptr(coef), L.ptr(side), L.ptr(cubic_q15),
                                      L.ptr(cubic_f32), L.stream_ptr())
    L.check(st, "mtlora_augment_batch")
    return outs


def _layout_weight(weight, bias, cdtype, col_index, n_cols, pad_rows):
    w = weight.detach().to(cdtype)
    if col_index is not None:
        w = w.new_zeros(w.shape[0], n_cols).index_copy(1, col_index, w)
    b = None if bias is None else bias.detach()
    if pad_rows:
        w = torch.cat([w, w.new_zeros(pad_rows, w.shape[1])], 0)
        b = None if b is None else torch.cat([b, b.new_zeros(pad_rows)], 0)
    return w.contiguous(), b


def _unlayout_grads(dw, db, col_index, pad_rows):
    if pad_rows:
        dw = None if dw is None else dw[:dw.shape[0] - pad_rows]
        db = None if db is None else db[:db.shape[0] - pad_rows].contiguous()
    if col_index is not None and dw is not None:
        dw = dw.index_select(1, col_index)
    elif dw is not None and pad_rows:
        dw = dw.contiguous()
    return dw, db


class SplitKLinearFn(torch.autograd.Function):

    @staticmethod
    def forward(ctx, x, weight, bias, splits: int, zero_bias_grad: bool, cdtype, col_index=None, n_cols=0, pad_rows=0):
        w, bl = _layout_weight(weight, bias, cdtype, col_index, n_cols, pad_rows)
        ctx.save_for_backward(x, w)
        ctx.wlayout = (col_index, pad_rows)
        ctx.has_bias = bias is not None
        ctx.splits = splits
        ctx.zero_bias_grad = zero_bias_grad
        ctx.wdtype = weight.dtype
        ctx.bdtype = None if bias is None else bias.dtype
        return torch.nn.functional.linear(x, w, None if bl is None else bl.to(cdtype))

    @staticmethod
    def backward(ctx, gy):
        x, w = ctx.saved_tensors
        gy = gy.contiguous()
        M, K = x.shape
        N = w.shape[0]
        S = ctx.splits
        dx = gy @ w if ctx.needs_input_grad[0] else None

        def wgrads():
            dw = None
            if ctx.needs_input_grad[1]:
                part = torch.bmm(gy.view(S, M // S, N).transpose(1, 2), x.view(S, M // S, K))
                dw = part.sum(0, dtype=torch.float32).to(ctx.wdtype)
            db = None
            if ctx.has_bias and ctx.needs_input_grad[2]:
                if ctx.zero_bias_grad:
                    db = torch.zeros(N, dtype=ctx.bdtype, device=gy.device)
                else:
                    db = column_sum(gy).to(ctx.bdtype)
            return _unlayout_grads(dw, db, *ctx.wlayout)

        dw, db = wgrads()
        return dx, dw, db, None, None, None, None, None, None


class PlainLinearFn(torch.autograd.Function):

    @staticmethod
    def forward(ctx, x, weight, bias, splits: int, zero_bias_grad: bool, cdtype, col_index=None, n_cols=0, pad_rows=0):
        L.require_gpu(x, weight)
        M, K = x.shape
        w, bias_l = _layout_weight(weight, bias, cdtype, col_index, n_cols, pad_rows)
        N = w.shape[0]
        meta = LinearMeta(K=K, N=N, r_s=0, r_t=(), scale_s=0.0, scale_t=(), mode=0, has_x_tasks=False, dropout_p=0.0, seed=0,
                          dtype=cdtype)
        d = meta.desc(M)
        lib = L.lib()
        ctx_bytes = _desc_bytes("ctx", lib.mtlora_linear_ctx_bytes, meta, M, d)
        if ctx_bytes < 0:
            raise RuntimeError(f"mtlora_amd: invalid plain-linear shape M={M} K={K} N={N}")
        ctxbuf = torch.empty(max(ctx_bytes, 16), dtype=torch.uint8, device=x.device)
        y = torch.empty((M, N), dtype=cdtype, device=x.device)
        bf = None if bias_l is None else bias_l.float().contiguous()
        st = lib.mtlora_linear_fwd(ctypes.byref(d), L.ptr(x), L.ptr_array(None), L.ptr(w), L.ptr(bf), L.ptr(None), L.ptr(None),
                                   L.ptr_array(None), L.ptr_array(None), L.ptr(y), L.ptr_array(None), L.ptr(ctxbuf), ctx_bytes,
                                   L.stream_ptr())
        L.check(st, "mtlora_linear_fwd (rank 0)")
        ctx.save_for_backward(x, w, ctxbuf)
        ctx.wlayout = (col_index, pad_rows)
        ctx.meta, ctx.splits, ctx.zero_bias_grad = meta, splits, zero_bias_grad
        ctx.has_bias, ctx.wdtype = bias is not None, weight.dtype
        ctx.bdtype = None if bias is None else bias.dtype
        return y

    @staticmethod
    def backward(ctx, gy):
        x, w, ctxbuf = ctx.saved_tensors
        gy = gy.contiguous()
        M, K = x.shape
        N = w.shape[0]
        S = ctx.splits
        dx = None
        if ctx.needs_input_grad[0]:
            d = ctx.meta.desc(M)
            lib = L.lib()
            sb = _desc_bytes("bwd", lib.mtlora_linear_bwd_scratch_bytes, ctx.meta, M, d)
            scratch = torch.empty(max(sb, 16), dtype=torch.uint8, device=x.device)
            wt = w.t().contiguous()
            dx = torch.empty((M, K), dtype=x.dtype, device=x.device)
            st = lib.mtlora_linear_bwd(ctypes.byref(d), L.ptr(x), L.ptr_array(None), L.ptr(wt), L.ptr(gy), L.ptr_array(None),
                                       L.ptr(ctxbuf), ctxbuf.numel(), L.ptr(dx), L.ptr_array(None), L.ptr(None), L.ptr(None),
                                       L.ptr_array(None), L.ptr_array(None), L.ptr(scratch), sb, L.stream_ptr())
            L.check(st, "mtlora_linear_bwd (rank 0)")
        def wgrads():
            dw = None
            if ctx.needs_input_grad[1]:
                if N <= 64:
                    dw = gemm_tn(gy, x).to(ctx.wdtype)
                else:
                    part = torch.bmm(gy.view(S, M // S, N).transpose(1, 2), x.view(S, M // S, K))
                    dw = part.sum(0, dtype=torch.float32).to(ctx.wdtype)
            db = None
            if ctx.has_bias and ctx.needs_input_grad[2]:
                if ctx.zero_bias_grad:
                    db = torch.zeros(N, dtype=ctx.bdtype, device=gy.device)
                else:
                    db = column_sum(gy).to(ctx.bdtype)
            return _unlayout_grads(dw, db, *ctx.wlayout)

        dw, db = wgrads()
        return dx, dw, db, None, None, None, None, None, None


def gemm_tn(a: torch.Tensor, b: torch.Tensor) -> torch.Tensor:
    L.require_gpu(a, b)
    if a.dtype != b.dtype or a.dim() != 2 or b.dim() != 2 or a.shape[0] != b.shape[0]:
        raise ValueError("gemm_tn: (M, Na) and (M, Nb) matrices of one dtype expected")
    a, b = a.contiguous(), b.contiguous()
    M, Na = a.shape
    Nb = b.shape[1]
    lib = L.lib()
    sb = lib.mtlora_gemm_tn_scratch_bytes(M, Na, Nb)
    if sb < 0:
        raise RuntimeError(f"mtlora_amd: invalid gemm_tn shape M={M} Na={Na} Nb={Nb}")
    scratch = torch.empty(sb, dtype=torch.uint8, device=a.device)
    out = torch.empty((Na, Nb), dtype=torch.float32, device=a.device)
    st = lib.mtlora_gemm_tn(L.ptr(a), L.ptr(b), L.ptr(out), M, Na, Nb, Na, Nb, _DT_CODE[a.dtype],
                            L.ptr(scratch), sb, L.stream_ptr())
    L.check(st, "mtlora_gemm_tn")
    return out


_PLAIN_VIA_KNT = os.environ.get("MTLORA_HEAD_GEMM", "knt") != "blas"


def _big_linear(x, weight, bias, S, feeds_batchnorm, cdtype, col_index=None, pad_rows=0):
    K, N = x.shape[1], weight.shape[0] + pad_rows
    if (_PLAIN_VIA_KNT and cdtype in _HOT_DTYPES and K % 8 == 0 and N % 8 == 0
            and x.dtype == cdtype):
        return PlainLinearFn.apply(x, weight, bias, S, feeds_batchnorm, cdtype, col_index, K, pad_rows)
    return SplitKLinearFn.apply(x, weight, bias, S, feeds_batchnorm, cdtype, col_index, K, pad_rows)


def linear_big_m(x: torch.Tensor, weight: torch.Tensor, bias: Optional[torch.Tensor],
                 feeds_batchnorm: bool = False, col_index: Optional[torch.Tensor] = None, pad_rows: int = 0) -> torch.Tensor:
    M = x.shape[0]
    if x.dim() == 2 and x.is_cuda and weight.requires_grad and torch.is_grad_enabled() and M >= 1 and x.is_contiguous():
        S = 1
        if M >= 16384:
            tiles = ((weight.shape[0] + 63) // 64) * ((weight.shape[1] + 63) // 64)
            S = 4
            while S < 64 and S * tiles < 2048 and M % (2 * S) == 0 and M // (2 * S) >= 1024:
                S *= 2
            if M % S:
                S = 1
        if torch.is_autocast_enabled("cuda"):
            dt = torch.get_autocast_dtype("cuda")
            with torch.autocast("cuda", enabled=False):
                return _big_linear(x.to(dt), weight, bias, S, feeds_batchnorm, dt, col_index, pad_rows)
        return _big_linear(x, weight, bias, S, feeds_batchnorm, x.dtype, col_index, pad_rows)
    if col_index is not None:
        weight = weight.new_zeros(weight.shape[0], x.shape[1]).index_copy(1, col_index, weight)
    if pad_rows:
        weight = torch.cat([weight, weight.new_zeros(pad_rows, weight.shape[1])], 0)
        bias = None if bias is None else torch.cat([bias, bias.new_zeros(pad_rows)], 0)
    return torch.nn.functional.linear(x, weight, bias)


def _pad4(c: int) -> int:
    return (c + 3) // 4 * 4


class ConcatUpsampleFn(torch.autograd.Function):

    @staticmethod
    def layout(channels):
        offs, o = [], 0
        for c in channels:
            offs.append(o)
            o += _pad4(c)
        return offs, (o + 7) // 8 * 8

    @staticmethod
    def forward(ctx, *maps):
        L.require_gpu(*maps)
        B, H, W, _ = maps[0].shape
        chans = [m.shape[3] for m in maps]
        offs, ld = ConcatUpsampleFn.layout(chans)
        dt = maps[0].dtype
        out = torch.empty(B * H * W, ld, dtype=dt, device=maps[0].device)
        o3 = out.view(B, H, W, ld)
        o3[..., :chans[0]].copy_(maps[0])
        lib = L.lib()
        end = chans[0]
        for i in range(1, len(maps)):
            if offs[i] > end:
                o3[..., end:offs[i]].zero_()
            m = maps[i].contiguous()
            _, h, w, C = m.shape
            if H % h or W % w or H // h != W // w or C % 4 or m.dtype != dt:
                raise RuntimeError("mtlora_amd: ConcatUpsampleFn needs integer scales, C % 4 == 0 and one dtype")
            st = lib.mtlora_upsample_cl_fwd(L.ptr(m), ctypes.c_void_p(out.data_ptr() + offs[i] * out.element_size()), B, h, w, C,
                                            H // h, ld, L.dtype_code(m), L.stream_ptr())
            L.check(st, "mtlora_upsample_cl_fwd")
            end = offs[i] + C
        if ld > end:
            o3[..., end:].zero_()
        ctx.shapes = [tuple(m.shape) for m in maps]
        ctx.offs, ctx.ld = offs, ld
        return out

    @staticmethod
    def backward(ctx, g):
        g = g.contiguous()
        B, H, W, C0 = ctx.shapes[0]
        ld = ctx.ld
        grads = [g.view(B, H, W, ld)[..., :C0]]
        lib = L.lib()
        for i in range(1, len(ctx.shapes)):
            _, h, w, C = ctx.shapes[i]
            d = torch.empty(ctx.shapes[i], dtype=g.dtype, device=g.device)
            st = lib.mtlora_upsample_cl_bwd(ctypes.c_void_p(g.data_ptr() + ctx.offs[i] * g.element_size()), L.ptr(d), B, h, w, C,
                                            H // h, ld, L.dtype_code(g), L.stream_ptr())
            L.check(st, "mtlora_upsample_cl_bwd")
            grads.append(d)
        return tuple(grads)


class BlockCall:
    __slots__ = ("has_norm1", "metas", "weights", "mask", "mask_ids", "H", "W", "num_heads", "window_size", "shift", "hidden",
                 "eps", "attn_scale", "mask_value", "factor_params", "norm_params", "desc", "params", "n_flat")

    def __init__(self, has_norm1, metas, weights, mask, mask_ids, H, W, num_heads, window_size, shift, hidden, eps, attn_scale,
                 factor_params, norm_params=(), mask_value=-100.0):
        self.has_norm1, self.metas, self.weights, self.mask, self.mask_ids = has_norm1, metas, weights, mask, mask_ids
        self.H, self.W, self.num_heads, self.window_size, self.shift, self.hidden = H, W, num_heads, window_size, shift, hidden
        self.eps, self.attn_scale, self.mask_value, self.factor_params = eps, attn_scale, mask_value, factor_params
        self.norm_params = tuple(norm_params)
        self.desc = self.params = None
        self.n_flat = 17 if has_norm1 else 15

    def build_desc(self, B: int, C: int, cdtype: torch.dtype, x_dtype: torch.dtype) -> "L.BlockDesc":
        d = L.BlockDesc()
        d.B, d.H, d.W, d.C, d.hidden = B, self.H, self.W, C, self.hidden
        d.num_heads, d.window_size, d.shift = self.num_heads, self.window_size, self.shift
        d.dtype, d.x_dtype, d.has_norm1 = _DT_CODE[cdtype], _DT_CODE[x_dtype], 1 if self.has_norm1 else 0
        d.eps1, d.eps2, d.eps_next = self.eps
        d.attn_scale, d.mask_value = self.attn_scale, self.mask_value
        M = B * self.H * self.W
        for i, m in enumerate(self.metas):
            d.lin[i] = m.desc(M)
        self.desc = d
        return d


_blk_bytes_cache: dict = {}


def _block_bytes(call: "BlockCall", d, B: int, C: int) -> Tuple[int, int, int]:
    key = (B, call.H, call.W, C, call.hidden, call.has_norm1, d.dtype, d.x_dtype, call.window_size, call.num_heads, call.shift,
           call.mask_ids is not None, tuple((m.r_s, m.packed is not None) for m in call.metas))
    v = _blk_bytes_cache.get(key)
    if v is None:
        lib = L.lib()
        v = (lib.mtlora_block_save_bytes(ctypes.byref(d)), lib.mtlora_block_fwd_tmp_bytes(ctypes.byref(d)),
             lib.mtlora_block_bwd_scratch_bytes(ctypes.byref(d)))
        if min(v) < 0:
            raise RuntimeError(f"mtlora_amd: invalid SwinTransformerBlock geometry B={B} H={call.H} W={call.W} C={C} hidden={call.hidden}")
        _blk_bytes_cache[key] = v
    return v


class SwinBlockRunFn(torch.autograd.Function):

    @staticmethod
    def forward(ctx, calls, x, normed, *flat):
        L.require_gpu(x, normed)
        lib = L.lib()
        B, _, C = x.shape
        M = x.numel() // C
        cdtype = calls[0].metas[0].dtype
        if not x.is_contiguous() or (normed is not None and (normed.dtype != cdtype or not normed.is_contiguous())):
            raise RuntimeError("mtlora_amd: SwinBlockRunFn needs contiguous inputs, norm1(x) in the compute dtype")
        stream = L.stream_ptr()
        dev = x.device
        tmp = None
        at = 0
        xs, ns, saves = [x], [normed], []
        for c in calls:
            t = flat[at:at + c.n_flat]
            at += c.n_flat
            for q in t:
                if q is not None and (q.device != dev or q.dtype != torch.float32 or not q.is_contiguous()):
                    raise RuntimeError("mtlora_amd: SwinBlockRunFn needs contiguous fp32 bias / DropPath / LayerNorm / factor tensors on the input's device")
# ... 106 lines not shown
```

mtlora_amd/lora.py:

```python
from __future__ import annotations

import math
import os
from typing import Any, Dict, Mapping, Optional, Tuple, Union

import torch
import torch.nn as nn

from . import functional as Fn

_MODES = ("matrix", "matrixv2", "add", "addition", "lora_only")


class LoRALayer(nn.Module):

    def __init__(self, r: int, lora_alpha: float, lora_dropout: float):
        super().__init__()
        assert r >= 0
        self.r = r
        self.lora_alpha = lora_alpha
        self.lora_dropout = nn.Dropout(p=lora_dropout) if lora_dropout > 0.0 else (lambda x: x)
        self.merged = False

    @property
# ... 203 lines not shown
            meta.packed = self._packed
        return meta

    def hid_call(self, dtype: torch.dtype, device):
        if not (self.r > 0 and self.tasks and self.shared_mode == "matrix" and not self.merged and hasattr(self, "lora_tasks_A")
                and hasattr(self, "lora_shared_A")):
            return None
        tasks = list(self.tasks)
        if isinstance(self.lora_shared_scale, torch.Tensor) or any(isinstance(self.lora_task_scale[t], torch.Tensor) for t in tasks):
            return None
        if self.linear.weight.requires_grad or (self.linear.bias is not None and self.linear.bias.requires_grad):
            return None
        if self.rank_aware_shared() or any(self._rank_aware(self._ranks[t], self.lora_task_scale[t]) for t in tasks):
            return None
        p = self.dropout_p if self.training else 0.0
        ss, st = float(self.lora_shared_scale), tuple(float(self.lora_task_scale[t]) for t in tasks)
        meta = Fn.LinearMeta(K=self.linear.in_features, N=self.linear.out_features, r_s=self.r, r_t=tuple(self._ranks[t] for t in tasks),
                             scale_s=ss, scale_t=st, mode=0, has_x_tasks=True, dropout_p=p, seed=Fn.next_seed() if p > 0 else 0, dtype=dtype)
        sig = (dtype, meta.r_s, meta.r_t, meta.scale_s, meta.scale_t, meta.mode, True, p, str(device))
        self._call_sig = sig
        if self._packed is not None and self._packed_sig == (sig, tuple(q._version for q in self._factor_params())):
            meta.packed = self._packed
        factors = (self.lora_shared_A, self.lora_shared_B, [self.lora_tasks_A[t] for t in tasks], [self.lora_tasks_B[t] for t in tasks])
        return meta, self._weights(dtype), factors

    def forward(self, x: torch.Tensor, x_tasks: Optional[Dict[str, torch.Tensor]] = None, gelu_gate=None, gelu_out: bool = False
                ) -> Tuple[torch.Tensor, Optional[Dict[str, torch.Tensor]]]:
        dtype = Fn.compute_dtype(x)
        wc, wt, bf = self._weights(dtype)
        has_lora = self.r > 0
        tasks = list(self.tasks) if (has_lora and self.tasks is not None) else []
        shared = has_lora and self.shared_mode in ("matrix", "matrixv2") and not self.merged
        p = self.dropout_p if (self.training and has_lora) else 0.0
        val = lambda s: float(s.detach().item()) if isinstance(s, torch.Tensor) else float(s)
        par = lambda s: s if isinstance(s, nn.Parameter) else None
        ss = self.lora_shared_scale if shared else 0.0
        st = [self.lora_task_scale[t] for t in tasks]
        ra_s = shared and self.rank_aware_shared()
        ra_t = [bool(tasks) and self._rank_aware(self._ranks[t], st[0]) for t in tasks]
        A_s, B_s = (self.lora_shared_A, self.lora_shared_B) if shared else (None, None)
        A_t, B_t = [self.lora_tasks_A[t] for t in tasks], [self.lora_tasks_B[t] for t in tasks]
        r_s, r_t = (self.r if shared else 0), [self._ranks[t] for t in tasks]
        vs, vt = val(ss), [val(s) for s in st]
        if ra_s or any(ra_t):
            K_, N_ = self.linear.in_features, self.linear.out_features
            if ra_s:
                (A_s,), (B_s,) = _delta_factors([A_s], [B_s], [vs], K_, N_)
                r_s, vs = min(K_, N_), 1.0
            idx = [i for i, f in enumerate(ra_t) if f]
            if idx:
                Ae, Be = _delta_factors([A_t[i] for i in idx], [B_t[i] for i in idx], [vt[i] for i in idx], K_, N_)
                for j, i in enumerate(idx):
                    A_t[i], B_t[i], r_t[i], vt[i] = Ae[j], Be[j], min(K_, N_), 1.0
        meta = Fn.LinearMeta(
            K=self.linear.in_features, N=self.linear.out_features,
            r_s=r_s, r_t=tuple(r_t), scale_s=vs, scale_t=tuple(vt),
            mode=1 if (self.shared_mode == "matrixv2" and tasks and not self.merged) else 0,
            has_x_tasks=bool(tasks) and x_tasks is not None, dropout_p=p, seed=Fn.next_seed() if p > 0 else 0,
            dtype=dtype, weight_requires_grad=self.linear.weight.requires_grad or (
                self.linear.bias is not None and self.linear.bias.requires_grad),
            n_scale_t=len(tasks) if (tasks and isinstance(st[0], nn.Parameter)) else 0)
        if has_lora and (ra_s or any(ra_t)):
            self._call_sig = None
        elif has_lora:
            sig = (dtype, meta.r_s, meta.r_t, meta.scale_s, meta.scale_t, meta.mode, meta.has_x_tasks, p, str(x.device))
            self._call_sig = sig
            if self._packed is not None and self._packed_sig == (sig, tuple(q._version for q in self._factor_params())):
                meta.packed = self._packed
        if gelu_out:
            if self.shared_mode == "addition":
                raise RuntimeError("mtlora_amd: gelu_out is not available with shared_mode='addition'")
            meta.gelu_out = True
        gates = []
        if gelu_gate is not None:
            gates = [gelu_gate[0]] + ([gelu_gate[1][t] for t in tasks] if meta.has_x_tasks else [])
            meta.n_gate = len(gates)
        args = [meta, x, wc, wt, bf, self.linear.weight, self.linear.bias, A_s, B_s, None if ra_s else par(ss)]
        if meta.has_x_tasks:
            args += [x_tasks[t] for t in tasks]
        args += A_t + B_t
        if meta.n_scale_t:
            args += st
        args += gates
        outs = Fn.MTLoRALinearFn.apply(*args)
        y = outs[0]
        if gelu_out:
            nt = len(tasks)
            return (y, {t: outs[1 + i] for i, t in enumerate(tasks)} if tasks else None,
                    outs[1 + nt], {t: outs[2 + nt + i] for i, t in enumerate(tasks)} if tasks else None)
        if not has_lora:
            return y, None
        y_tasks = {t: outs[1 + i] for i, t in enumerate(tasks)} if tasks else None
        if self.shared_mode == "addition":
            tot = torch.stack(list(y_tasks.values()), 0).sum(0).float()
            y = y + nn.functional.layer_norm(tot, (tot.shape[-1],), self.lora_norm.weight.float(),
                                             self.lora_norm.bias.float(), self.lora_norm.eps).to(y.dtype)
        return y, y_tasks


class FactorPacker:

    def __init__(self, model: nn.Module):
        self.layers = [m for m in model.modules() if isinstance(m, MTLoRALinear) and m.r > 0]
        self._table = None
        self._table_key = None
        self._tables = {}

    def _eligible(self, m: "MTLoRALinear") -> bool:
        if m._call_sig is None or m.merged:
            return False
        if isinstance(m.lora_shared_scale, torch.Tensor):
            return False
        if m.tasks is not None and isinstance(m.lora_task_scale, nn.ParameterDict):
            return False
        return all(q.dtype == torch.float32 and q.is_contiguous() and q.is_cuda for q in m._factor_params())

    def refresh(self) -> int:
        for m in self.layers:
            m.__dict__.pop("_fp_cache", None)
        todo = [m for m in self.layers if self._eligible(m)]
        if not todo:
            return 0
        key = tuple((id(m), m._call_sig) + tuple(q.data_ptr() for q in m._factor_params()) for m in todo)
        if key != self._table_key and key in self._tables:
            self._table = self._tables[key]
            self._table_key = key
            for tb in self._table:
                for ent in tb.keep:
                    ent[6]._packed = ent[5]
        elif key != self._table_key:
            by_dtype = {}
            for m in todo:
                dtype, r_s, r_t, scale_s, scale_t, mode, has_xt, p, _dev = m._call_sig
                meta = Fn.LinearMeta(K=m.linear.in_features, N=m.linear.out_features, r_s=r_s, r_t=r_t, scale_s=scale_s, scale_t=scale_t,
                                     mode=mode, has_x_tasks=has_xt, dropout_p=p, seed=0, dtype=dtype)
                dev = m._factor_params()[0].device
                need = Fn.packed_bytes(meta)
                m._packed = torch.empty(need, dtype=torch.uint8, device=dev)
                shared = r_s > 0
                tasks = list(m.tasks) if (m.tasks is not None and len(r_t) > 0) else []
                ent = (meta, m.lora_shared_A if shared else None, m.lora_shared_B if shared else None,
                       [m.lora_tasks_A[t] for t in tasks], [m.lora_tasks_B[t] for t in tasks], m._packed, m)
                by_dtype.setdefault((dtype, str(dev)), []).append(ent)
            self._table = [Fn.PackTable(ents, ents[0][5].device, dt) for (dt, _), ents in by_dtype.items()]
            self._table_key = key
            self._tables[key] = self._table
        for tb in self._table:
            tb.pack()
        for m in todo:
            m._packed_sig = (m._call_sig, tuple(q._version for q in m._factor_params()))
        return len(todo)


def mark_only_lora_as_trainable(model: nn.Module, bias: str = "none", freeze_patch_embed: bool = False,
                                freeze_norm: bool = False, free_relative_bias: bool = False,
                                freeze_downsample_reduction=False) -> None:
    keep = [("lora_", True), ("patch_embed", not freeze_patch_embed), ("norm", not freeze_norm),
            ("downsample.reduction", not freeze_downsample_reduction),
            ("relative_position_bias_table", not free_relative_bias)]
    for name, p in model.named_parameters():
        if not any(on and key in name for key, on in keep):
            p.requires_grad = False
    if bias == "none":
        return
    if bias == "all":
        for name, p in model.named_parameters():
            if "bias" in name:
                p.requires_grad = True
    elif bias == "lora_only":
        for m in model.modules():
            if isinstance(m, LoRALayer) and getattr(m, "bias", None) is not None:
                m.bias.requires_grad = True
    else:
        raise NotImplementedError


def lora_filter(key: str, value: Any) -> bool:
    return "lora_" in key


def map_old_state_dict_weights(state_dict: Dict, mapping: Mapping, prefix: str, split_qkv: bool = False) -> Dict:
    missing = []
    for old, new in mapping.items():
        src = prefix + old
        if src not in state_dict:
            missing.append(old)
            continue
        w = state_dict.pop(src)
        dst = prefix + new
        tail = ".".join(dst.split(".")[-4:])
        if split_qkv and tail in ("attn.qkv.linear.weight", "attn.qkv.linear.bias"):
            kind = tail.split(".")[-1]
            stem = ".".join(dst.split(".")[:-2])
            for nm, part in zip("qkv", torch.chunk(w, chunks=3)):
                state_dict[f"{stem}.{nm}.linear.{kind}"] = part
        else:
            state_dict[dst] = w
    if missing:
        print(f"WARNING: The following keys from the checkpoint were not mapped: {missing}")
    return state_dict
```

mtlora_amd/mtl_harness.py:

```python
from __future__ import annotations

import contextlib
import ctypes
import os
from typing import Dict, List, Mapping, Optional, Sequence

import torch
import torch.nn as nn
import torch.nn.functional as F

from . import functional as Fn
from .functional import BatchNormReluFn, UpsampleLossFn
from .lora import MTLoRALinear, mark_only_lora_as_trainable
from .optim import FusedAdamW, accumulation_steps_of
from .swin_transformer_mtlora import SwinTransformerMTLoRA

NUM_OUTPUT = {"semseg": 21, "normals": 3, "sal": 1, "human_parts": 7, "depth": 1, "edge": 1}
EDGE_POS_WEIGHT = 0.95
NYUD4 = ("semseg", "depth", "normals", "edge")
NYUD_NUM_OUTPUT = {"semseg": 40}
LOSS_WEIGHTS = {"depth": 1.0, "semseg": 1.0, "human_parts": 2.0, "sal": 5.0, "edge": 50.0, "normals": 10.0}


def is_synthetic_task(t: str) -> bool:
# ... 210 lines not shown
    if task == "normals":
        mask = (label != 255).to(out.dtype)
        on = out / (torch.norm(out, p=2, dim=1, keepdim=True) + 1e-12)
        return ((on - label).abs() * mask).sum() / mask.sum().clamp_min(1e-6)
    if task == "sal":
        labels = (label >= 0.5).to(out.dtype)
        w = (1.0 - labels).sum() / labels.numel()
        gz = (out >= 0).to(out.dtype)
        lv = out * (labels - gz) - torch.log(1 + torch.exp(out - 2 * out * gz))
        return (w * (-(labels * lv)).sum() + (1 - w) * (-((1.0 - labels) * lv)).sum()) / labels.numel()
    if task == "depth":
        mask = (label != 255).to(out.dtype)
        return ((out - label).abs() * mask).sum() / mask.sum().clamp_min(1.0)
    if task == "edge":
        labels = (label >= 0.5).to(out.dtype)
        gz = (out >= 0).to(out.dtype)
        lv = out * (labels - gz) - torch.log(1 + torch.exp(out - 2 * out * gz))
        return (EDGE_POS_WEIGHT * (-(labels * lv)).sum() + (1 - EDGE_POS_WEIGHT) * (-((1.0 - labels) * lv)).sum()) / labels.numel()
    raise NotImplementedError(task)


class MultiTaskLoss(nn.Module):

    def __init__(self, tasks: Sequence[str], loss_weights: Optional[Mapping[str, float]] = None):
        super().__init__()
        self.tasks = list(tasks)
        self.loss_weights = dict(loss_weights or {t: loss_weight(t) for t in tasks})

    def forward(self, pred, gt):
        per = {t: task_loss(t, pred[t], gt[t]) for t in self.tasks}
        total = torch.stack([self.loss_weights[t] * per[t] for t in self.tasks]).sum()
        per["total"] = total
        return total, per

    FUSED_KIND = {"semseg": "softmax", "human_parts": "softmax", "normals": "normals", "sal": "balanced_bce",
                  "depth": "l1_masked", "edge": "balanced_bce"}

    def task_low(self, t, lo, lab):
        h, w = lo.shape[1:3]
        H, W = lab.shape[-2:]
        kind = self.FUSED_KIND.get(task_kind(t))
        if kind is not None and lo.is_cuda and H % h == 0 and W % w == 0 and H // h == W // w:
            if task_kind(t) == "edge":
                return UpsampleLossFn.apply(kind, lo, lab, H // h, 255.0, EDGE_POS_WEIGHT)
            return UpsampleLossFn.apply(kind, lo, lab, H // h)
        return task_loss(t, F.interpolate(lo.permute(0, 3, 1, 2), (H, W), mode="bilinear"), lab)

    def combine(self, per):
        per = dict(per)
        total = torch.stack([self.loss_weights[t] * per[t] for t in self.tasks]).sum()
        per["total"] = total
        return total, per

    def forward_low(self, low, gt):
        return self.combine({t: self.task_low(t, low[t], gt[t]) for t in self.tasks})


def build_model(img_size=448, tasks=("semseg", "normals", "sal", "human_parts"), embed_dim=96, depths=(2, 2, 6, 2),
                num_heads=(3, 6, 12, 24), r_shared=64, r_task=4, drop_path_rate=0.2, lora_b_std=0.02, seed=0,
                freeze=True, num_outputs: Optional[Mapping[str, int]] = None, **mt_over) -> MultiTaskSwin:
    torch.manual_seed(seed)
    mt = mtlora_namespace(tasks, r_shared, r_task, n_stages=len(depths), **mt_over)
    bb = SwinTransformerMTLoRA(img_size=img_size, patch_size=4, in_chans=3, num_classes=0, embed_dim=embed_dim,
                               depths=list(depths), num_heads=list(num_heads), window_size=7, mlp_ratio=4.0,
                               qkv_bias=True, drop_rate=0.0, drop_path_rate=drop_path_rate, ape=False, patch_norm=True,
                               tasks=list(tasks), mtlora=mt)
    model = MultiTaskSwin(bb, tasks, {t: int((num_outputs or {}).get(t, num_output(t))) for t in tasks})
    if lora_b_std > 0:
        with torch.no_grad():
            for n, p in model.named_parameters():
                if "lora_" in n and "_B" in n:
                    p.normal_(0.0, lora_b_std)
    if freeze:
        mark_only_lora_as_trainable(model.backbone, bias="none")
    return model


def build_optimizer(model: nn.Module, lr=5e-4, weight_decay=0.05, fused: Optional[bool] = None,
                    capturable: bool = False, impl: str = "torch") -> torch.optim.Optimizer:
    if impl not in ("torch", "hip"):
        raise ValueError(f"build_optimizer: impl must be 'torch' or 'hip', got {impl!r}")
    decay, no_decay = [], []
    for n, p in model.named_parameters():
        if not p.requires_grad:
            continue
        if p.ndim == 1 or n.endswith(".bias") or "relative_position_bias_table" in n or "absolute_pos_embed" in n:
            no_decay.append(p)
        else:
            decay.append(p)
    groups = [{"params": decay}, {"params": no_decay, "weight_decay": 0.0}]
    if impl == "hip":
        return FusedAdamW(groups, lr=lr, betas=(0.9, 0.999), eps=1e-8, weight_decay=weight_decay, capturable=bool(capturable))
    if fused is None:
        fused = all(p.is_cuda for p in decay + no_decay)
    return torch.optim.AdamW(groups, lr=lr, betas=(0.9, 0.999), eps=1e-8, weight_decay=weight_decay, fused=fused,
                             capturable=bool(capturable and fused))


def synthetic_batch(B: int, S: int, tasks: Sequence[str], seed: int, device="cpu", num_outputs: Optional[Mapping[str, int]] = None):
    g = torch.Generator(device="cpu").manual_seed(seed)
    img = torch.randn(B, 3, S, S, generator=g)
    tg = {}
    for t in tasks:
        k = task_kind(t)
        if k in ("semseg", "human_parts"):
            lab = torch.randint(0, int((num_outputs or {}).get(t, NUM_OUTPUT[k])), (B, 1, S, S), generator=g).float()
            lab[torch.rand(B, 1, S, S, generator=g) < 0.05] = 255.0
        elif k == "sal":
            lab = (torch.rand(B, 1, S, S, generator=g) < 0.3).float()
        elif k == "normals":
            lab = F.normalize(torch.randn(B, 3, S, S, generator=g), dim=1)
            ign = (torch.rand(B, 1, S, S, generator=g) < 0.05).expand(B, 3, S, S)
            lab = torch.where(ign, torch.full_like(lab, 255.0), lab)
        elif k == "depth":
            lab = torch.rand(B, 1, S, S, generator=g) * 10
        elif k == "edge":
            lab = (torch.rand(B, 1, S, S, generator=g) < 0.1).float()
        else:
            raise NotImplementedError(t)
        tg[t] = lab.to(device)
    return img.to(device), tg


_FACTOR_STREAM = os.environ.get("MTLORA_FACTOR_STREAM", "1") != "0"
_factor_streams: Dict[str, "torch.cuda.Stream"] = {}


def _factor_side_stream(device):
    if not _FACTOR_STREAM or not _streams_allowed():
        return None
    key = str(device)
    if key not in _factor_streams:
        _factor_streams[key] = torch.cuda.Stream(device=device)
    return _factor_streams[key]


_PACK_ONCE = os.environ.get("MTLORA_PACK_ONCE", "1") != "0"


class _NoPacker:
    def refresh(self):
        return 0


def _factor_packer(model):
    pk = getattr(model, "_mtlora_factor_packer", None)
    if pk is None:
        from .lora import FactorPacker
        pk = FactorPacker(model) if _PACK_ONCE else _NoPacker()
        object.__setattr__(model, "_mtlora_factor_packer", pk)
    return pk


def train_step(model, criterion, optimizer, images, targets, clip_grad: float = 5.0, reducer=None,
               amp_dtype: Optional[torch.dtype] = torch.bfloat16, fused_loss: bool = True, loss_scaler=None,
               update_grad: bool = True):
    fused_opt = isinstance(optimizer, FusedAdamW)
    if loss_scaler is not None and not fused_opt:
        raise TypeError("train_step: loss_scaler needs the HIP optimizer (build_optimizer(impl='hip'))")
    def fwd():
        if fused_loss:
            if isinstance(model, MultiTaskSwin):
                return criterion.combine(model(images, upsample=False,
                                               per_task_fn=lambda t, lo: criterion.task_low(t, lo, targets[t])))
            return criterion.forward_low(model(images, upsample=False), targets)
        return criterion(model(images), targets)

    if images.is_cuda:
        Fn.droppath_begin_step(images.device)
        _factor_packer(model).refresh()
    try:
        if amp_dtype is not None:
            with torch.autocast("cuda", dtype=amp_dtype):
                loss, per = fwd()
        else:
            loss, per = fwd()
    finally:
        Fn.droppath_end_step()
    side = _factor_side_stream(images.device) if images.is_cuda else None
    if reducer is not None:
        extra = list(model._streams) if (isinstance(model, MultiTaskSwin) and getattr(model, "_streams", None)) else []
        reducer.extra_streams = extra + ([side] if side is not None else [])
        reducer.prepare()
    Fn.set_factor_stream(side)
    try:
        (loss if loss_scaler is None else loss_scaler.scale(loss)).backward()
    finally:
        Fn.set_factor_stream(None)
    if side is not None:
        torch.cuda.current_stream(images.device).wait_stream(side)
        Fn.factor_stream_joined()
    if reducer is not None:
        reducer.finish()
    if not update_grad:
        return loss.detach(), None
    if fused_opt:
        norm = optimizer.clip_and_step(clip_grad or None, loss_scaler)
        optimizer.zero_grad(set_to_none=True)
        return loss.detach(), norm
    params = [p for g in optimizer.param_groups for p in g["params"] if p.grad is not None]
    norm = torch.nn.utils.clip_grad_norm_(params, clip_grad, foreach=True) if clip_grad else None
    optimizer.step()
    optimizer.zero_grad(set_to_none=True)
    return loss.detach(), norm


def validate_step(model, criterion, meter, images, targets, amp_dtype: Optional[torch.dtype] = torch.bfloat16):
    was_training = model.training
    model.eval()
    try:
        with torch.no_grad():
            ctx = (torch.autocast("cuda", dtype=amp_dtype) if (amp_dtype is not None and images.is_cuda)
                   else contextlib.nullcontext())
            with ctx:
                if isinstance(model, MultiTaskSwin):
                    conc = images.is_cuda and _TASK_STREAMS and len(model.tasks) > 1 and _streams_allowed()
                    per = model(images, upsample=False, concurrent=conc,
                                per_task_fn=lambda t, lo: meter.update_task_low(t, lo, targets[t]))
                else:
                    low = model(images, upsample=False)
                    per = {t: meter.update_task_low(t, low[t], targets[t]) for t in criterion.tasks}
            return criterion.combine({t: per[t].float() for t in criterion.tasks})
    finally:
        model.train(was_training)


def validate(model, batches, criterion=None, meter=None, database: str = "PASCALContext",
             amp_dtype: Optional[torch.dtype] = torch.bfloat16, verbose: bool = False):
    from .evaluation import PerformanceMeter
    tasks = list(model.tasks)
    criterion = criterion if criterion is not None else MultiTaskLoss(tasks)
    meter = meter if meter is not None else PerformanceMeter(tasks, database)
    total, n = None, 0
    for images, targets in batches:
        loss, _ = validate_step(model, criterion, meter, images, targets, amp_dtype)
        total = loss.double() if total is None else total + loss.double()
        n += 1
    scores = meter.get_score(verbose)
    return scores, (float(total) / n if n else float("nan"))


def predict_step(model, images, tasks=None, uint8=False, amp_dtype=torch.bfloat16):
    from .evaluation import get_output_low
    wanted = list(model.tasks if tasks is None else tasks)
    H, W = images.shape[-2:]

    def finish(t, lo):
        if t not in wanted:
            return lo
        h, w = lo.shape[1:3]
        if H % h or W % w or H // h != W // w:
            raise RuntimeError(f"mtlora_amd: predict_step needs an integer scale, got {(h, w)} -> {(H, W)} for {t}")
        return get_output_low(lo, t, H // h, uint8)

    was_training = model.training
    model.eval()
    try:
        with torch.no_grad():
            ctx = (torch.autocast("cuda", dtype=amp_dtype) if (amp_dtype is not None and images.is_cuda)
                   else contextlib.nullcontext())
            with ctx:
                if isinstance(model, MultiTaskSwin):
                    conc = images.is_cuda and _TASK_STREAMS and len(model.tasks) > 1 and _streams_allowed()
                    per = model(images, upsample=False, concurrent=conc, per_task_fn=finish)
                else:
                    low = model(images, upsample=False)
                    per = {t: finish(t, low[t]) for t in wanted}
            return {t: per[t] for t in wanted}
    finally:
        model.train(was_training)


def predict(model, batches, tasks=None, uint8=False, amp_dtype=torch.bfloat16):
    for batch in batches:
        images = batch[0] if isinstance(batch, (tuple, list)) else batch
        yield predict_step(model, images, tasks, uint8, amp_dtype)


class GraphedTrainStep:

    SEED_STEP = 0x1E3779B97F4A7C15

    def __init__(self, model, criterion, optimizer, images, targets, clip_grad: float = 5.0, reducer=None,
                 amp_dtype: Optional[torch.dtype] = torch.bfloat16, fused_loss: bool = True, warmup: int = 3, loss_scaler=None,
                 accumulation_steps: int = 1):
        self.accumulation_steps = accumulation_steps_of(accumulation_steps)
        if self.accumulation_steps > 1 and reducer is not None:
            raise ValueError("GraphedTrainStep: accumulation_steps > 1 with a reducer is not supported (the all-reduce would have to "
                             "sit between two graphs on every k-th call only); use train_step(..., reducer=, update_grad=)")
        self.fused_opt = isinstance(optimizer, FusedAdamW)
        if self.accumulation_steps > 1 and not self.fused_opt:
            raise TypeError("GraphedTrainStep: accumulation_steps > 1 needs the HIP optimizer (build_optimizer(impl='hip', "
                            "capturable=True)): the decision to step is taken on the device by its kernels")
        if self.fused_opt and not optimizer._capturable:
            raise TypeError("GraphedTrainStep: a FusedAdamW inside the graph must be built with capturable=True "
                            "(build_optimizer(impl='hip', capturable=True)): its hyper-parameters travel in the launch arguments, "
                            "which a replay cannot follow")
        if loss_scaler is not None and not self.fused_opt:
            raise TypeError("GraphedTrainStep: loss_scaler needs the HIP optimizer (build_optimizer(impl='hip', capturable=True))")
        self.model, self.criterion, self.optimizer = model, criterion, optimizer
        self.images, self.targets = images, targets
        self.clip_grad, self.reducer, self.amp_dtype, self.fused_loss = clip_grad, reducer, amp_dtype, fused_loss
        self.loss_scaler, self.grad_norm = loss_scaler, None
        self._calls, self.updated = 0, False
        if self.accumulation_steps > 1:
            optimizer.prepare_accumulation()
        if loss_scaler is not None:
            loss_scaler._lazy_init(images.device)
        self.graphed, self.why = False, ""
        self.seed = torch.zeros(1, dtype=torch.int64, device=images.device)
        Fn.set_seed_offset(self.seed)
        self.g_bwd = self.g_opt = None
        self.loss = None
        try:
            self._capture(warmup)
            self.graphed = True
            ok, why = self._replays_reproduce()
            if not ok:
                raise RuntimeError(why)
        except Exception as e:
            self.graphed = False
            self.why = f"{type(e).__name__}: {e}"
            torch.cuda.synchronize()
            self.g_bwd = self.g_opt = None
            if self.fused_opt:
                optimizer.reset_capture()
            optimizer.zero_grad(set_to_none=True)
            self._calls = 0
            Fn.set_seed_offset(None)

    def _replays_reproduce(self):
        params = [p for g in self.optimizer.param_groups for p in g["params"]]
        bufs = [b for b in self.model.buffers() if b.is_floating_point()]

        extra = [self.optimizer._ctrl, self.optimizer._exp_avg, self.optimizer._exp_avg_sq] if self.fused_opt else []
        if self.loss_scaler is not None:
            extra += [self.loss_scaler._scale, self.loss_scaler._growth_tracker]
        acc = self.optimizer._acc if self.accumulation_steps > 1 else None
        if acc is not None:
            extra += [acc, self.optimizer._accum_norm]

        def snap():
            st = {} if self.fused_opt else {
                id(p): {k: (v.clone() if torch.is_tensor(v) else v) for k, v in self.optimizer.state.get(p, {}).items()}
                for p in params}
            return ([p.detach().clone() for p in params], [b.clone() for b in bufs], st, torch.cuda.get_rng_state(),
                    self.seed.clone(), [t.clone() for t in extra])

        def restore(s):
            with torch.no_grad():
                torch._foreach_copy_([p.data for p in params], s[0])
                if bufs:
                    torch._foreach_copy_(bufs, s[1])
                for p in params:
                    for k, v in s[2].get(id(p), {}).items():
                        if torch.is_tensor(v):
                            self.optimizer.state[p][k].copy_(v)
                self.seed.copy_(s[4])
                for t, v in zip(extra, s[5]):
                    t.copy_(v)
            torch.cuda.set_rng_state(s[3])

        if self.fused_opt:
            self.optimizer.push_hyperparameters()
        torch.cuda.synchronize()
        s0 = snap()
        seen, acc_seen = [], []
        for _ in range(3):
            restore(s0)
            self.g_bwd.replay()
            if self.g_opt is not None:
                self.reducer.all_reduce_packed()
                self.g_opt.replay()
            torch.cuda.synchronize()
            seen.append((self.loss.clone(), torch.stack([p.detach().double().sum() for p in params]).sum()))
            if acc is not None:
                acc_seen.append(acc.view(torch.int32).sum())
        restore(s0)
        if self.fused_opt:
            self.optimizer.bump_versions()
        for l, c in seen[1:]:
            if not (torch.equal(l, seen[0][0]) and torch.equal(c, seen[0][1]) and torch.isfinite(l).all()):
                return False, ("graph replays from identical state differ (loss %r vs %r, parameter sums %r); running eagerly.  A "
                               "loss that differs from the second replay on points at a captured small memset (an ATen reduction), "
                               "which does not replay on this ROCm stack; an equal loss with differing parameters at a gradient "
                               "that is summed with atomics (an ATen backward such as bilinear interpolation)"
                               % (seen[0][0].item(), l.item(), [c.item() for _, c in seen]))
        if any(not torch.equal(a, acc_seen[0]) for a in acc_seen[1:]):
            return False, ("graph replays from identical state accumulate different gradients (checksums %r); running eagerly"
                           % [a.item() for a in acc_seen])
        return True, ""

    def _forward_backward(self):
        self.seed.add_(self.SEED_STEP)
        if self.images.is_cuda:
            _factor_packer(self.model).refresh()
        ctx = (torch.autocast("cuda", dtype=self.amp_dtype, cache_enabled=False) if self.amp_dtype is not None
               else contextlib.nullcontext())
        with ctx:
            if self.fused_loss and isinstance(self.model, MultiTaskSwin):
                loss, _ = self.criterion.combine(self.model(
                    self.images, upsample=False, per_task_fn=lambda t, lo: self.criterion.task_low(t, lo, self.targets[t])))
            elif self.fused_loss:
                loss, _ = self.criterion.forward_low(self.model(self.images, upsample=False), self.targets)
            else:
                loss, _ = self.criterion(self.model(self.images), self.targets)
        side = _factor_side_stream(self.images.device) if self.images.is_cuda else None
        if self.reducer is not None:
            extra = list(self.model._streams) if (isinstance(self.model, MultiTaskSwin) and getattr(self.model, "_streams", None)) else []
            self.reducer.extra_streams = extra + ([side] if side is not None else [])
            self.reducer.prepare(defer=True)
        Fn.set_factor_stream(side)
        try:
            (loss if self.loss_scaler is None else self.loss_scaler.scale(loss)).backward()
        finally:
            Fn.set_factor_stream(None)
        if side is not None:
            torch.cuda.current_stream(self.images.device).wait_stream(side)
            Fn.factor_stream_joined()
        if self.reducer is not None:
            self.reducer.flush_packs()
        return loss.detach()

    def _optimize(self, accumulation_steps: int = 1):
        if self.reducer is not None:
            self.reducer.unpack()
        if self.fused_opt:
            self.grad_norm = self.optimizer.clip_and_step(self.clip_grad or None, self.loss_scaler, accumulation_steps)
            self.optimizer.zero_grad(set_to_none=True)
            return
        params = [p for g in self.optimizer.param_groups for p in g["params"] if p.grad is not None]
        if self.clip_grad:
            torch.nn.utils.clip_grad_norm_(params, self.clip_grad, foreach=True)
        self.optimizer.step()
        self.optimizer.zero_grad(set_to_none=True)

    def _eager(self, update_grad: bool = True):
        loss = self._forward_backward()
        if self.reducer is not None:
            self.reducer.all_reduce_packed()
        if update_grad:
            self._optimize()
        return loss

    def _count(self) -> bool:
        self._calls += 1
        self.updated = self._calls % self.accumulation_steps == 0
        return self.updated

    def _capture(self, warmup: int):
        side = torch.cuda.Stream()
        side.wait_stream(torch.cuda.current_stream())
        with torch.cuda.stream(side):
            for _ in range(max(2, warmup)):
                self._eager()
        torch.cuda.current_stream().wait_stream(side)
        torch.cuda.synchronize()
        self.optimizer.zero_grad(set_to_none=True)
        self.g_bwd = torch.cuda.CUDAGraph()
        if self.reducer is None:
            with torch.cuda.graph(self.g_bwd):
                self.loss = self._forward_backward()
                self._optimize(self.accumulation_steps)
        else:
            with torch.cuda.graph(self.g_bwd):
                self.loss = self._forward_backward()
            self.g_opt = torch.cuda.CUDAGraph()
            with torch.cuda.graph(self.g_opt, pool=self.g_bwd.pool()):
                self._optimize()
        torch.cuda.synchronize()

    def __call__(self):
        updated = self._count()
        if not self.graphed:
            return self._eager(updated)
        if self.fused_opt:
            self.optimizer.push_hyperparameters()
        self.g_bwd.replay()
        if self.g_opt is not None:
            self.reducer.all_reduce_packed()
            self.g_opt.replay()
        if self.fused_opt:
            self.optimizer.bump_versions(updated)
        return self.loss
```

Baseline: 1148 images/sec.

## Batch-pack plain-linear weights once per step and fuse weight-grad reduction

```diff
diff --git a/include/mtlora_hip.h b/include/mtlora_hip.h
--- a/include/mtlora_hip.h
+++ b/include/mtlora_hip.h
@@ -114,6 +114,18 @@
 int64_t mtlora_gemm_tn_scratch_bytes(int64_t M, int Na, int Nb);
 int mtlora_gemm_tn(const void* a, const void* b, float* out, int64_t M, int Na, int Nb, int64_t lda, int64_t ldb,
                    int dtype, void* scratch, int64_t scratch_bytes, void* stream);
+
+#define MTLORA_PLAIN_DB_NONE 0
+#define MTLORA_PLAIN_DB_ZERO 1
+#define MTLORA_PLAIN_DB_COLSUM 2
+int64_t mtlora_plain_pack_entry_bytes(void);
+int mtlora_plain_pack_entry(const float* weight, const float* bias, const int32_t* col_inv, int rows, int cols, int n_cols, int pad_rows,
+                            void* W, void* Wt, float* bias_out, void* entry_host);
+int mtlora_plain_pack_table(const void* table_dev, int n_entries, int dtype, void* stream);
+int64_t mtlora_plain_wgrad_scratch_bytes(int64_t M, int N, int K, int native, int db_mode);
+int mtlora_plain_wgrad(const void* gy, const void* x, const void* partials, int64_t M, int N, int K, int dtype, const int32_t* col_inv,
+                       int cols, int pad_rows, int splits, int db_mode, float* dW, float* db, void* scratch, int64_t scratch_bytes,
+                       void* stream);
 
 typedef struct mtlora_attn_desc {
     int64_t B;
diff --git a/mtlora_amd/_lib.py b/mtlora_amd/_lib.py
--- a/mtlora_amd/_lib.py
+++ b/mtlora_amd/_lib.py
@@ -76,6 +76,8 @@
 ADAMW_GROUPS_DEV_BYTES = 1152
 ADAMW_CTRL_MICRO, ADAMW_CTRL_UPDATED = 5, 6
 ADAMW_MAX_ACCUM_STEPS = 1 << 24
+
+PLAIN_DB_NONE, PLAIN_DB_ZERO, PLAIN_DB_COLSUM = 0, 1, 2
 
 PROF_KINDS = 24
 
@@ -114,6 +116,12 @@
     "mtlora_gemm_tn_scratch_bytes": (c_int64, [c_int64, c_int, c_int]),
     "mtlora_gemm_tn": (c_int, [c_void_p, c_void_p, c_void_p, c_int64, c_int, c_int, c_int64, c_int64, c_int, c_void_p, c_int64,
                                c_void_p]),
+    "mtlora_plain_pack_entry_bytes": (c_int64, []),
+    "mtlora_plain_pack_entry": (c_int, [c_void_p, c_void_p, c_void_p, c_int, c_int, c_int, c_int, c_void_p, c_void_p, c_void_p, c_void_p]),
+    "mtlora_plain_pack_table": (c_int, [c_void_p, c_int, c_int, c_void_p]),
+    "mtlora_plain_wgrad_scratch_bytes": (c_int64, [c_int64, c_int, c_int, c_int, c_int]),
+    "mtlora_plain_wgrad": (c_int, [c_void_p, c_void_p, c_void_p, c_int64, c_int, c_int, c_int, c_void_p, c_int, c_int, c_int, c_int,
+                                   c_void_p, c_void_p, c_void_p, c_int64, c_void_p]),
     "mtlora_linear_fwd_gelu": (c_int, [POINTER(LinearDesc), c_void_p, POINTER(c_void_p), c_void_p, c_void_p, c_void_p, c_void_p,
                                        POINTER(c_void_p), POINTER(c_void_p), c_void_p, POINTER(c_void_p), c_void_p,
                                        POINTER(c_void_p), c_void_p, c_int64, c_void_p]),
diff --git a/mtlora_amd/csrc/build.py b/mtlora_amd/csrc/build.py
--- a/mtlora_amd/csrc/build.py
+++ b/mtlora_amd/csrc/build.py
@@ -4,7 +4,7 @@
 from concurrent.futures import ThreadPoolExecutor
 
 HERE = os.path.dirname(os.path.abspath(__file__))
-SOURCES = ["window_process.hip", "linear.hip", "attention.hip", "glue.hip", "layernorm.hip", "loss.hip", "metrics.hip", "predict.hip", "upsample.hip", "reduce.hip", "selftest.hip", "block.hip", "hid.hip", "optim.hip", "ingest.hip", "augment.hip"]
+SOURCES = ["window_process.hip", "linear.hip", "attention.hip", "glue.hip", "layernorm.hip", "loss.hip", "metrics.hip", "predict.hip", "upsample.hip", "reduce.hip", "selftest.hip", "block.hip", "hid.hip", "optim.hip", "ingest.hip", "augment.hip", "plain.hip"]
 LIB = os.path.join(HERE, "libmtlora_hip.so")
 FLAGS = ["--offload-arch=gfx950", "-O3", "-std=c++17", "-fPIC", "-Wno-unused-value", "-Wno-unused-result"]
 
diff --git a/mtlora_amd/csrc/common.h b/mtlora_amd/csrc/common.h
--- a/mtlora_amd/csrc/common.h
+++ b/mtlora_amd/csrc/common.h
@@ -344,6 +344,8 @@
     PK_NT_PLAIN_FWD = 17,
     PK_NT_PLAIN_DX = 18,
     PK_TN_PLAIN = 19,
+    PK_PLAIN_PACK = 20,
+    PK_PLAIN_WGRAD = 21,
     PK_COUNT = 24
 };
 int mtl_prof_start(int kind, double alg_bytes, hipStream_t s, double s8d_bytes = 0.0, double flops = 0.0);
diff --git a/mtlora_amd/csrc/internal.h b/mtlora_amd/csrc/internal.h
--- a/mtlora_amd/csrc/internal.h
+++ b/mtlora_amd/csrc/internal.h
@@ -13,6 +13,12 @@
                                              int64_t B, int64_t M, int64_t C, int x_dtype, int dy_dtype, void* scratch,
                                              int64_t scratch_bytes, const void* dx_addend, int phase, void* stream);
 
+#define MTLI_TN_A 64
+#define MTLI_TN_B 256
+MTL_INTERNAL int mtli_gemm_tn_partials(const void* a, const void* b, int64_t M, int Na, int Nb, int dtype, void* scratch,
+                                       int64_t scratch_bytes, int* plan, void* stream);
+MTL_INTERNAL int mtli_colsum(const void* x, int64_t M, int64_t N, int dtype, float* out, int n_out, void* scratch, void* stream);
+
 struct HidLaunch;
 struct HidParams;
 struct HidRedParams;
diff --git a/mtlora_amd/csrc/linear.hip b/mtlora_amd/csrc/linear.hip
--- a/mtlora_amd/csrc/linear.hip
+++ b/mtlora_amd/csrc/linear.hip
@@ -2054,18 +2054,19 @@
     return (int64_t)ta * tb * ns * TN_TILE * 4 + 256;
 }
 
-int mtlora_gemm_tn(const void* a, const void* b, float* out, int64_t M, int Na, int Nb, int64_t lda, int64_t ldb,
-                   int dtype, void* scratch, int64_t scratch_bytes, void* stream) {
+static int gemm_tn_run(const void* a, const void* b, float* out, int64_t M, int Na, int Nb, int64_t lda, int64_t ldb, int dtype,
+                       void* scratch, int64_t scratch_bytes, bool reduce, int* plan, void* stream) {
     if (dtype != MTLORA_F32 && dtype != MTLORA_BF16 && dtype != MTLORA_F16) return MTLORA_ERR_DTYPE;
     const int vec = dtype == MTLORA_F32 ? 4 : 8;
     if (M < 0 || M >= ((int64_t)1 << 31) || Na <= 0 || Nb <= 0 || lda < Na || ldb < Nb) return MTLORA_ERR_SHAPE;
     if (Na % vec || Nb % vec || lda % vec || ldb % vec) return MTLORA_ERR_ALIGN;
     if (Na > 1024) return MTLORA_ERR_UNSUPPORTED;
-    if (!out || !scratch || (M > 0 && (!a || !b))) return MTLORA_ERR_NULL;
+    if ((reduce && !out) || !scratch || (M > 0 && (!a || !b))) return MTLORA_ERR_NULL;
     if (misaligned(a) || misaligned(b) || misaligned(scratch) || ((uintptr_t)out & 3u)) return MTLORA_ERR_ALIGN;
     if (scratch_bytes < mtlora_gemm_tn_scratch_bytes(M, Na, Nb) - 256) return MTLORA_ERR_WORKSPACE;
     hipStream_t s = (hipStream_t)stream;
     if (M == 0) {
+        if (!reduce) return MTLORA_ERR_SHAPE;
         mtl_zero_async(out, (size_t)Na * Nb * 4, s);
         return MTLORA_OK;
     }
@@ -2104,9 +2105,25 @@
         else
             hipLaunchKernelGGL(k_tn<bf16>, dim3((unsigned)tp.nsplit, (unsigned)(ta * tb), 1), dim3(256), 0, s, tp);
     }
+    if (plan) plan[0] = ta, plan[1] = tb, plan[2] = tp.nsplit;
+    if (!reduce) {
+        MTL_CHECK_LAUNCH();
+        return MTLORA_OK;
+    }
     MtlProfScope prof(PK_REDUCE, 0.0, s);
     hipLaunchKernelGGL(k_tn_reduce, dim3(TN_TILE / 1024, (unsigned)(ta * tb), 1), dim3(256 * TN_RG), 0, s, tp);
     MTL_CHECK_LAUNCH();
     return MTLORA_OK;
 }
-}
+
+int mtlora_gemm_tn(const void* a, const void* b, float* out, int64_t M, int Na, int Nb, int64_t lda, int64_t ldb,
+                   int dtype, void* scratch, int64_t scratch_bytes, void* stream) {
+    return gemm_tn_run(a, b, out, M, Na, Nb, lda, ldb, dtype, scratch, scratch_bytes, true, nullptr, stream);
+}
+
+static_assert(TN_A == MTLI_TN_A && TN_B == MTLI_TN_B, "internal.h states the tile of the partials");
+int mtli_gemm_tn_partials(const void* a, const void* b, int64_t M, int Na, int Nb, int dtype, void* scratch, int64_t scratch_bytes,
+                          int* plan, void* stream) {
+    return gemm_tn_run(a, b, nullptr, M, Na, Nb, Na, Nb, dtype, scratch, scratch_bytes, false, plan, stream);
+}
+}
diff --git a/mtlora_amd/csrc/plain.hip b/mtlora_amd/csrc/plain.hip
--- /dev/null
+++ b/mtlora_amd/csrc/plain.hip
@@ -0,0 +1,300 @@
+#include <string.h>
+
+#include "common.h"
+#include "internal.h"
+
+namespace {
+
+struct PlainPackEntry {
+    const float* w;
+    const float* bias;
+    const int32_t* col_inv;
+    void* W;
+    void* Wt;
+    float* b;
+    int32_t rows, cols, n_cols, N;
+};
+
+template <typename T>
+__device__ __forceinline__ T pp_round(float v);
+template <>
+__device__ __forceinline__ bf16 pp_round<bf16>(float v) {
+    const uint32_t u = __builtin_bit_cast(uint32_t, v);
+    const uint16_t h = (v != v) ? (uint16_t)0x7FC0u : (uint16_t)((u + (((u >> 16) & 1u) + 0x7FFFu)) >> 16);
+    return __builtin_bit_cast(bf16, h);
+}
+template <>
+__device__ __forceinline__ f16 pp_round<f16>(float v) {
+    return (f16)v;
+}
+
+constexpr int PP_T = 64;
+
+template <typename T>
+__global__ __launch_bounds__(256) void k_plain_pack(const PlainPackEntry* __restrict__ table) {
+    __shared__ __attribute__((aligned(16))) T tile[PP_T][PP_T + 8];
+    const PlainPackEntry e = table[blockIdx.y];
+    const int tid = threadIdx.x;
+    const int tiles_k = (e.n_cols + PP_T - 1) / PP_T, tiles = ((e.N + PP_T - 1) / PP_T) * tiles_k;
+    T* __restrict__ W = reinterpret_cast<T*>(e.W);
+    T* __restrict__ Wt = reinterpret_cast<T*>(e.Wt);
+    const bool vec = ((e.N | e.n_cols) & 7) == 0;
+    if (blockIdx.x == 0 && e.b)
+        for (int n = tid; n < e.N; n += 256) e.b[n] = n < e.rows ? e.bias[n] : 0.f;
+    for (int t = blockIdx.x; t < tiles; t += gridDim.x) {
+        const int n0 = (t / tiles_k) * PP_T, k0 = (t % tiles_k) * PP_T;
+        {
+            const int c = tid & 63, k = k0 + c;
+            int src = -1;
+            if (k < e.n_cols) src = e.col_inv ? e.col_inv[k] : k;
+#pragma unroll 4
+            for (int i = 0; i < PP_T / 4; ++i) {
+                const int r = (tid >> 6) + 4 * i, n = n0 + r;
+                const float v = (src >= 0 && n < e.rows) ? e.w[(int64_t)n * e.cols + src] : 0.f;
+                tile[r][c] = pp_round<T>(v);
+            }
+        }
+        __syncthreads();
+        if (vec) {
+#pragma unroll
+            for (int h = 0; h < 2; ++h) {
+                const int q = tid + 256 * h, r = q >> 3, v = q & 7;
+                const int n = n0 + r, k = k0 + v * 8;
+                if (n < e.N && k < e.n_cols)
+                    *reinterpret_cast<u32x4*>(W + (int64_t)n * e.n_cols + k) = *reinterpret_cast<const u32x4*>(&tile[r][v * 8]);
+                const int kt = k0 + r, nt = n0 + v * 8;
+                if (kt < e.n_cols && nt < e.N) {
+                    Vec16<T> o;
+#pragma unroll
+                    for (int j = 0; j < 8; ++j) o.e[j] = tile[v * 8 + j][r];
+                    *reinterpret_cast<u32x4*>(Wt + (int64_t)kt * e.N + nt) = o.raw;
+                }
+            }
+        } else {
+            const int c = tid & 63;
+            for (int i = 0; i < PP_T / 4; ++i) {
+                const int r = (tid >> 6) + 4 * i;
+                if (n0 + r < e.N && k0 + c < e.n_cols) W[(int64_t)(n0 + r) * e.n_cols + k0 + c] = tile[r][c];
+                if (k0 + r < e.n_cols && n0 + c < e.N) Wt[(int64_t)(k0 + r) * e.N + n0 + c] = tile[c][r];
+            }
+        }
+        __syncthreads();
+    }
+}
+
+struct PlainFinish {
+    int rows, cols, K;
+    const int32_t* col_inv;
+    float* dW;
+    float* db_zero;
+};
+
+__device__ __forceinline__ void pf_zero_db(const PlainFinish& F, bool first_block) {
+    if (first_block && F.db_zero)
+        for (int n = threadIdx.x; n < F.rows; n += blockDim.x) F.db_zero[n] = 0.f;
+}
+
+constexpr int PF_RG = 4;
+__global__ __launch_bounds__(256 * PF_RG) void k_plain_finish_tiles(const PlainFinish F, const float* __restrict__ part, int tiles_b,
+                                                                     int nsplit) {
+    constexpr int TILE = MTLI_TN_A * MTLI_TN_B;
+    __shared__ f32x4 sm[PF_RG][256];
+    pf_zero_db(F, blockIdx.x == 0 && blockIdx.y == 0);
+    const int tb = blockIdx.y;
+    const int t = threadIdx.x & 255, grp = threadIdx.x >> 8;
+    const int e0 = blockIdx.x * 1024 + t * 4;
+    const int a = e0 / MTLI_TN_B, b0 = tb * MTLI_TN_B + e0 % MTLI_TN_B;
+    const bool live = a < F.rows && b0 < F.K;
+    f32x4 acc[4];
+#pragma unroll
+    for (int u = 0; u < 4; ++u) acc[u] = f32x4{0.f, 0.f, 0.f, 0.f};
+    if (live) {
+        const float* src = part + (int64_t)tb * TILE + e0;
+        const int64_t stride = (int64_t)tiles_b * TILE;
+        int sp = grp;
+        for (; sp + 3 * PF_RG < nsplit; sp += 4 * PF_RG) {
+#pragma unroll
+            for (int u = 0; u < 4; ++u) acc[u] += *reinterpret_cast<const f32x4*>(src + (int64_t)(sp + u * PF_RG) * stride);
+        }
+        for (; sp < nsplit; sp += PF_RG) acc[0] += *reinterpret_cast<const f32x4*>(src + (int64_t)sp * stride);
+    }
+    sm[grp][t] = (acc[0] + acc[1]) + (acc[2] + acc[3]);
+    __syncthreads();
+    if (grp != 0 || !live) return;
+    f32x4 tsum = sm[0][t];
+#pragma unroll
+    for (int g = 1; g < PF_RG; ++g) tsum += sm[g][t];
+#pragma unroll
+    for (int e = 0; e < 4; ++e)
+        if (b0 + e < F.K) {
+            const int c = F.col_inv ? F.col_inv[b0 + e] : b0 + e;
+            if (c >= 0) F.dW[(int64_t)a * F.cols + c] = tsum[e];
+        }
+}
+
+template <typename T, int V>
+__global__ __launch_bounds__(256) void k_plain_finish_parts(const PlainFinish F, const T* __restrict__ part, int S, int N) {
+    pf_zero_db(F, blockIdx.x == 0);
+    const int kv = F.K / V;
+    const int64_t idx = (int64_t)blockIdx.x * 256 + threadIdx.x;
+    if (idx >= (int64_t)F.rows * kv) return;
+    const int n = (int)(idx / kv), k = (int)(idx % kv) * V;
+    const T* src = part + (int64_t)n * F.K + k;
+    const int64_t stride = (int64_t)N * F.K;
+    float acc[4][V];
+#pragma unroll
+    for (int u = 0; u < 4; ++u)
+#pragma unroll
+        for (int e = 0; e < V; ++e) acc[u][e] = 0.f;
+    auto add = [&](int u, int s) __attribute__((always_inline)) {
+        if constexpr (V == 8) {
+            const Vec16<T> q = mtl_ld16<T>(src + (int64_t)s * stride);
+#pragma unroll
+            for (int e = 0; e < 8; ++e) acc[u][e] += mtl_to_f32(q.e[e]);
+        } else {
+            acc[u][0] += mtl_to_f32(src[(int64_t)s * stride]);
+        }
+    };
+    int s = 0;
+    for (; s + 3 < S; s += 4) {
+#pragma unroll
+        for (int u = 0; u < 4; ++u) add(u, s + u);
+    }
+    for (int u = 0; s < S; ++s, ++u) add(u, s);
+#pragma unroll
+    for (int e = 0; e < V; ++e) {
+        const float v = ((acc[0][e] + acc[1][e]) + acc[2][e]) + acc[3][e];
+        const int c = F.col_inv ? F.col_inv[k + e] : k + e;
+        if (c >= 0) F.dW[(int64_t)n * F.cols + c] = v;
+    }
+}
+
+inline bool pp_mis16(const void* p) { return ((uintptr_t)p & 15u) != 0; }
+inline bool pp_mis4(const void* p) { return ((uintptr_t)p & 3u) != 0; }
+
+int64_t colsum_bytes(int N) { return mtlora_colsum_scratch_bytes(1, N); }
+
+}
+
+extern "C" {
+
+int64_t mtlora_plain_pack_entry_bytes(void) { return (int64_t)sizeof(PlainPackEntry); }
+
+int mtlora_plain_pack_entry(const float* weight, const float* bias, const int32_t* col_inv, int rows, int cols, int n_cols, int pad_rows,
+                            void* W, void* Wt, float* bias_out, void* entry_host) {
+    if (rows <= 0 || cols <= 0 || n_cols <= 0 || pad_rows < 0 || (int64_t)rows + pad_rows > (1 << 24) || n_cols > (1 << 24))
+        return MTLORA_ERR_SHAPE;
+    if (col_inv ? cols > n_cols : cols != n_cols) return MTLORA_ERR_SHAPE;
+    if (!weight || !W || !Wt || !entry_host || (bias != nullptr) != (bias_out != nullptr)) return MTLORA_ERR_NULL;
+    if (pp_mis4(weight) || pp_mis4(bias) || pp_mis4(col_inv) || pp_mis4(bias_out) || pp_mis16(W) || pp_mis16(Wt)) return MTLORA_ERR_ALIGN;
+    PlainPackEntry e;
+    memset(&e, 0, sizeof(e));
+    e.w = weight;
+    e.bias = bias;
+    e.col_inv = col_inv;
+    e.W = W;
+    e.Wt = Wt;
+    e.b = bias_out;
+    e.rows = rows;
+    e.cols = cols;
+    e.n_cols = n_cols;
+    e.N = rows + pad_rows;
+    memcpy(entry_host, &e, sizeof(e));
+    return MTLORA_OK;
+}
+
+int mtlora_plain_pack_table(const void* table_dev, int n_entries, int dtype, void* stream) {
+    if (dtype != MTLORA_BF16 && dtype != MTLORA_F16) return MTLORA_ERR_DTYPE;
+    if (n_entries <= 0 || n_entries > 65535) return MTLORA_ERR_SHAPE;
+    if (!table_dev) return MTLORA_ERR_NULL;
+    if (((uintptr_t)table_dev & 7u) != 0) return MTLORA_ERR_ALIGN;
+    hipStream_t s = (hipStream_t)stream;
+    MtlProfScope prof(PK_PLAIN_PACK, 0.0, s);
+    const dim3 g(32, (unsigned)n_entries);
+    if (dtype == MTLORA_F16)
+        hipLaunchKernelGGL(k_plain_pack<f16>, g, dim3(256), 0, s, reinterpret_cast<const PlainPackEntry*>(table_dev));
+    else
+        hipLaunchKernelGGL(k_plain_pack<bf16>, g, dim3(256), 0, s, reinterpret_cast<const PlainPackEntry*>(table_dev));
+    MTL_CHECK_LAUNCH();
+    return MTLORA_OK;
+}
+
+static int wgrad_check(int64_t M, int N, int K, int dtype, int splits, int db_mode, int native) {
+    if (dtype != MTLORA_BF16 && dtype != MTLORA_F16) return MTLORA_ERR_DTYPE;
+    if (M <= 0 || M >= ((int64_t)1 << 31) || N <= 0 || K <= 0 || N > (1 << 20) || K > (1 << 20)) return MTLORA_ERR_SHAPE;
+    if (splits <= 0 || splits > 65535 || M % splits) return MTLORA_ERR_SHAPE;
+    if (db_mode < MTLORA_PLAIN_DB_NONE || db_mode > MTLORA_PLAIN_DB_COLSUM) return MTLORA_ERR_UNSUPPORTED;
+    if (db_mode == MTLORA_PLAIN_DB_COLSUM && dtype != MTLORA_BF16) return MTLORA_ERR_DTYPE;
+    if (native && N > MTLI_TN_A) return MTLORA_ERR_UNSUPPORTED;
+    if ((native && (N % 8 || K % 8)) || (db_mode == MTLORA_PLAIN_DB_COLSUM && N % 8)) return MTLORA_ERR_ALIGN;
+    return MTLORA_OK;
+}
+
+int64_t mtlora_plain_wgrad_scratch_bytes(int64_t M, int N, int K, int native, int db_mode) {
+    if (M <= 0 || N <= 0 || K <= 0) return -1;
+    int64_t b = 256;
+    if (native) b += mtlora_gemm_tn_scratch_bytes(M, N, K);
+    if (db_mode == MTLORA_PLAIN_DB_COLSUM) b += colsum_bytes(N);
+    return b;
+}
+
+int mtlora_plain_wgrad(const void* gy, const void* x, const void* partials, int64_t M, int N, int K, int dtype, const int32_t* col_inv,
+                       int cols, int pad_rows, int splits, int db_mode, float* dW, float* db, void* scratch, int64_t scratch_bytes,
+                       void* stream) {
+    const int native = partials == nullptr;
+    int st = wgrad_check(M, N, K, dtype, splits, db_mode, native);
+    if (st != MTLORA_OK) return st;
+    const int rows = N - pad_rows;
+    if (pad_rows < 0 || rows <= 0 || cols <= 0 || (col_inv ? cols > K : cols != K)) return MTLORA_ERR_SHAPE;
+    if (!gy || !dW || (native && !x) || (db_mode != MTLORA_PLAIN_DB_NONE && !db)) return MTLORA_ERR_NULL;
+    const bool need_scratch = native || db_mode == MTLORA_PLAIN_DB_COLSUM;
+    if (need_scratch && !scratch) return MTLORA_ERR_NULL;
+    if (pp_mis16(gy) || pp_mis16(x) || pp_mis16(partials) || pp_mis16(scratch) || pp_mis4(dW) || pp_mis4(db) || pp_mis4(col_inv))
+        return MTLORA_ERR_ALIGN;
+    if (need_scratch && scratch_bytes < mtlora_plain_wgrad_scratch_bytes(M, N, K, native, db_mode)) return MTLORA_ERR_WORKSPACE;
+    hipStream_t s = (hipStream_t)stream;
+
+    PlainFinish F;
+    F.rows = rows;
+    F.cols = cols;
+    F.K = K;
+    F.col_inv = col_inv;
+    F.dW = dW;
+    F.db_zero = db_mode == MTLORA_PLAIN_DB_ZERO ? db : nullptr;
+    unsigned char* sc = reinterpret_cast<unsigned char*>(scratch);
+    if (native) {
+        const int64_t tn_bytes = mtlora_gemm_tn_scratch_bytes(M, N, K);
+        int plan[3];
+        st = mtli_gemm_tn_partials(gy, x, M, N, K, dtype, sc, tn_bytes, plan, stream);
+        if (st != MTLORA_OK) return st;
+        sc += mtl_round_up(tn_bytes, 256);
+        mtl_prof_tag("tiles M%lld N%d K%d", (long long)M, N, K);
+        MtlProfScope prof(PK_PLAIN_WGRAD, 0.0, s);
+        hipLaunchKernelGGL(k_plain_finish_tiles, dim3(MTLI_TN_A * MTLI_TN_B / 1024, (unsigned)plan[1], 1), dim3(256 * PF_RG), 0, s, F,
+                           reinterpret_cast<const float*>(scratch), plan[1], plan[2]);
+    } else {
+        mtl_prof_tag("parts S%d N%d K%d", splits, N, K);
+        MtlProfScope prof(PK_PLAIN_WGRAD, 2.0 * splits * (double)N * K, s);
+        const bool v8 = K % 8 == 0;
+        const unsigned g = (unsigned)mtl_ceil_div((int64_t)rows * (v8 ? K / 8 : K), 256);
+        if (dtype == MTLORA_F16) {
+            if (v8)
+                hipLaunchKernelGGL((k_plain_finish_parts<f16, 8>), dim3(g), dim3(256), 0, s, F, reinterpret_cast<const f16*>(partials), splits, N);
+            else
+                hipLaunchKernelGGL((k_plain_finish_parts<f16, 1>), dim3(g), dim3(256), 0, s, F, reinterpret_cast<const f16*>(partials), splits, N);
+        } else {
+            if (v8)
+                hipLaunchKernelGGL((k_plain_finish_parts<bf16, 8>), dim3(g), dim3(256), 0, s, F, reinterpret_cast<const bf16*>(partials), splits, N);
+            else
+                hipLaunchKernelGGL((k_plain_finish_parts<bf16, 1>), dim3(g), dim3(256), 0, s, F, reinterpret_cast<const bf16*>(partials), splits, N);
+        }
+    }
+    if (db_mode == MTLORA_PLAIN_DB_COLSUM) {
+        st = mtli_colsum(gy, M, N, dtype, db, rows, sc, stream);
+        if (st != MTLORA_OK) return st;
+    }
+    MTL_CHECK_LAUNCH();
+    return MTLORA_OK;
+}
+
+}
diff --git a/mtlora_amd/csrc/reduce.hip b/mtlora_amd/csrc/reduce.hip
--- a/mtlora_amd/csrc/reduce.hip
+++ b/mtlora_amd/csrc/reduce.hip
@@ -1,4 +1,5 @@
 #include "common.h"
+#include "internal.h"
 
 namespace {
 
@@ -42,7 +43,7 @@
 }
 
 constexpr int RD_RW = 16;
-__global__ __launch_bounds__(64 * RD_RW) void k_colsum_combine(const float* part, float* out, int nblk, int N, float scale) {
+__global__ __launch_bounds__(64 * RD_RW) void k_colsum_combine(const float* part, float* out, int nblk, int N, int n_out, float scale) {
     __shared__ float sm[RD_RW][64];
     const int lane = threadIdx.x & 63, wave = threadIdx.x >> 6;
     const int c = blockIdx.x * 64 + lane;
@@ -59,7 +60,7 @@
     }
     sm[wave][lane] = (a0 + a1) + (a2 + a3);
     __syncthreads();
-    if (wave == 0 && c < N) {
+    if (wave == 0 && c < n_out) {
         float t = 0.f;
 #pragma unroll
         for (int w = 0; w < RD_RW; ++w) t += sm[w][lane];
@@ -124,7 +125,12 @@
     if (!x || !out || !scratch) return MTLORA_ERR_NULL;
     if (((uintptr_t)x | (uintptr_t)scratch) & 15u) return MTLORA_ERR_ALIGN;
     if (scratch_bytes < mtlora_colsum_scratch_bytes(M, N)) return MTLORA_ERR_WORKSPACE;
+    return mtli_colsum(x, M, N, dtype, out, (int)N, scratch, stream);
+}
+
+int mtli_colsum(const void* x, int64_t M, int64_t N, int dtype, float* out, int n_out, void* scratch, void* stream) {
     hipStream_t s = (hipStream_t)stream;
+    const int ve = dtype == MTLORA_F32 ? 4 : 8;
     const int nvec = (int)(N / ve);
     const int rps = nvec >= 256 ? 1 : 256 / nvec;
     int64_t g = mtl_ceil_div(M, (int64_t)rps * 8);
@@ -135,8 +141,8 @@
         hipLaunchKernelGGL(k_colsum_part<float>, dim3((unsigned)g), dim3(256), 0, s, reinterpret_cast<const float*>(x), M, (int)N, part);
     else
         hipLaunchKernelGGL(k_colsum_part<bf16>, dim3((unsigned)g), dim3(256), 0, s, reinterpret_cast<const bf16*>(x), M, (int)N, part);
-    hipLaunchKernelGGL(k_colsum_combine, dim3((unsigned)mtl_ceil_div(N, 64)), dim3(64 * RD_RW), 0, s, (const float*)part, out, (int)g,
-                       (int)N, 1.f);
+    hipLaunchKernelGGL(k_colsum_combine, dim3((unsigned)mtl_ceil_div(n_out, 64)), dim3(64 * RD_RW), 0, s, (const float*)part, out, (int)g,
+                       (int)N, n_out, 1.f);
     MTL_CHECK_LAUNCH();
     return MTLORA_OK;
 }
diff --git a/mtlora_amd/csrc/selftest.hip b/mtlora_amd/csrc/selftest.hip
--- a/mtlora_amd/csrc/selftest.hip
+++ b/mtlora_amd/csrc/selftest.hip
@@ -175,6 +175,8 @@
         case PK_NT_PLAIN_FWD: return "k_nt:plain_fwd";
         case PK_NT_PLAIN_DX: return "k_nt:plain_dX";
         case PK_TN_PLAIN: return "k_tn:plain_dW";
+        case PK_PLAIN_PACK: return "k_plain_pack";
+        case PK_PLAIN_WGRAD: return "k_plain_wgrad";
         default: return "";
     }
 }
diff --git a/mtlora_amd/functional.py b/mtlora_amd/functional.py
--- a/mtlora_amd/functional.py
+++ b/mtlora_amd/functional.py
@@ -1485,12 +1485,128 @@
     return dw, db
 
 
+_PLAIN_PACK = os.environ.get("MTLORA_PLAIN_PACK", "1") != "0"
+_PACK_DTYPES = (torch.bfloat16, torch.float16)
+_plain_epoch = 0
+
+
+class PlainSlot:
+    __slots__ = ("cdtype", "shape", "offset", "bias", "col_index", "n_cols", "pad_rows", "W", "Wt", "b", "stamp")
+
+    def current_stamp(self, base):
+        b = self.bias
+        return (base.data_ptr(), base._version, 0 if b is None else b.data_ptr(), 0 if b is None else b._version)
+
+
+def col_inverse(col_index: torch.Tensor, n_cols: int) -> torch.Tensor:
+    inv = getattr(col_index, "_mtlora_inv", None)
+    if inv is None or inv.shape[0] != n_cols or inv.device != col_index.device:
+        inv = torch.full((n_cols,), -1, dtype=torch.int32, device=col_index.device)
+        inv[col_index] = torch.arange(col_index.numel(), dtype=torch.int32, device=col_index.device)
+        col_index._mtlora_inv = inv
+    return inv
+
+
+def _plain_lookup(weight, bias, cdtype, col_index, n_cols, pad_rows):
+    global _plain_epoch
+    if not _PLAIN_PACK or cdtype not in _PACK_DTYPES or weight.dtype != torch.float32 or not weight.is_contiguous():
+        return None, False
+    if bias is not None and (bias.dtype != torch.float32 or bias._base is not None or not bias.is_contiguous()):
+        return None, False
+    base = weight._base if weight._base is not None else weight
+    if not isinstance(base, torch.nn.Parameter):
+        return None, False
+    key = (cdtype, tuple(weight.shape), weight.storage_offset(), None if bias is None else id(bias),
+           None if col_index is None else id(col_index), n_cols, pad_rows)
+    slots = getattr(base, "_mtlora_plain", None)
+    if slots is None:
+        slots = base._mtlora_plain = {}
+    slot = slots.get(key)
+    if slot is None:
+        slot = slots[key] = PlainSlot()
+        slot.cdtype, slot.shape, slot.offset = cdtype, tuple(weight.shape), weight.storage_offset()
+        slot.bias, slot.col_index, slot.n_cols, slot.pad_rows = bias, col_index, n_cols, pad_rows
+        slot.W = slot.Wt = slot.b = slot.stamp = None
+        _plain_epoch += 1
+        return slot, False
+    return slot, slot.stamp is not None and slot.stamp == slot.current_stamp(base)
+
+
+def invalidate_plain_packs(model) -> None:
+    for p in model.parameters():
+        for slot in getattr(p, "_mtlora_plain", {}).values():
+            slot.stamp = None
+
+
+class PlainPackTable:
+
+    def __init__(self, entries, device, dtype: torch.dtype):
+        lib = L.lib()
+        eb = lib.mtlora_plain_pack_entry_bytes()
+        host = (ctypes.c_ubyte * (eb * max(len(entries), 1)))()
+        self.keep = [(p, s, s.W, s.Wt, s.b) for p, s in entries]
+        for i, (p, s) in enumerate(entries):
+            rows, cols = s.shape
+            inv = None if s.col_index is None else col_inverse(s.col_index, s.n_cols)
+            st = lib.mtlora_plain_pack_entry(ctypes.c_void_p(p.data_ptr() + 4 * s.offset), L.ptr(s.bias), L.ptr(inv), rows, cols, s.n_cols,
+                                             s.pad_rows, L.ptr(s.W), L.ptr(s.Wt), L.ptr(s.b), ctypes.byref(host, i * eb))
+            L.check(st, "mtlora_plain_pack_entry")
+        self.n = len(entries)
+        self.dtype_code = _DT_CODE[dtype]
+        self.table = torch.frombuffer(host, dtype=torch.uint8).clone().to(device)
+
+    def pack(self) -> None:
+        L.check(L.lib().mtlora_plain_pack_table(L.ptr(self.table), self.n, self.dtype_code, L.stream_ptr()), "mtlora_plain_pack_table")
+
+
+def plain_wgrad(gy, x, part, col_index, cols: int, pad_rows: int, splits: int, db_mode: int):
+    M, N = gy.shape
+    K = x.shape[1]
+    lib = L.lib()
+    native = part is None
+    sb = lib.mtlora_plain_wgrad_scratch_bytes(M, N, K, int(native), db_mode)
+    if sb < 0:
+        raise RuntimeError(f"mtlora_amd: invalid plain_wgrad shape M={M} N={N} K={K}")
+    scratch = torch.empty(sb, dtype=torch.uint8, device=gy.device) if (native or db_mode == L.PLAIN_DB_COLSUM) else None
+    rows = N - pad_rows
+    dw = torch.empty((rows, cols), dtype=torch.float32, device=gy.device)
+    db = torch.empty(rows, dtype=torch.float32, device=gy.device) if db_mode != L.PLAIN_DB_NONE else None
+    inv = None if col_index is None else col_inverse(col_index, K)
+    st = lib.mtlora_plain_wgrad(L.ptr(gy), L.ptr(x), L.ptr(part), M, N, K, _DT_CODE[gy.dtype], L.ptr(inv), cols, pad_rows, splits, db_mode,
+                                L.ptr(dw), L.ptr(db), L.ptr(scratch), sb, L.stream_ptr())
+    L.check(st, "mtlora_plain_wgrad")
+    return dw, db
+
+
+def _plain_wgrads(ctx, gy, x, N, K, narrow_native: bool):
+    col_index, pad_rows = ctx.wlayout
+    M, S = x.shape[0], ctx.splits
+    want_db = ctx.has_bias and ctx.needs_input_grad[2]
+    db_mode = L.PLAIN_DB_NONE
+    if want_db and ctx.zero_bias_grad:
+        db_mode = L.PLAIN_DB_ZERO
+    elif want_db and N % 8 == 0 and gy.dtype == torch.bfloat16:
+        db_mode = L.PLAIN_DB_COLSUM
+    part = None
+    if not (narrow_native and N <= 64):
+        part = torch.bmm(gy.view(S, M // S, N).transpose(1, 2), x.view(S, M // S, K))
+    dw, db = plain_wgrad(gy, x, part, col_index, ctx.wcols, pad_rows, S, db_mode)
+    if want_db and db_mode == L.PLAIN_DB_NONE:
+        db = _unlayout_grads(None, column_sum(gy).to(ctx.bdtype), col_index, pad_rows)[1]
+    return dw, db
+
+
 class SplitKLinearFn(torch.autograd.Function):
 
     @staticmethod
-    def forward(ctx, x, weight, bias, splits: int, zero_bias_grad: bool, cdtype, col_index=None, n_cols=0, pad_rows=0):
-        w, bl = _layout_weight(weight, bias, cdtype, col_index, n_cols, pad_rows)
+    def forward(ctx, x, weight, bias, splits: int, zero_bias_grad: bool, cdtype, col_index=None, n_cols=0, pad_rows=0, plain=None):
+        slot, packed = plain if plain is not None else (None, False)
+        if packed:
+            w, bl = slot.W, slot.b
+        else:
+            w, bl = _layout_weight(weight, bias, cdtype, col_index, n_cols, pad_rows)
         ctx.save_for_backward(x, w)
+        ctx.plain, ctx.wcols = slot is not None, weight.shape[1]
         ctx.wlayout = (col_index, pad_rows)
         ctx.has_bias = bias is not None
         ctx.splits = splits
@@ -1507,6 +1623,9 @@
         N = w.shape[0]
         S = ctx.splits
         dx = gy @ w if ctx.needs_input_grad[0] else None
+        if ctx.plain and ctx.needs_input_grad[1]:
+            dw, db = _plain_wgrads(ctx, gy, x, N, K, narrow_native=False)
+            return dx, dw, db, None, None, None, None, None, None, None
 
         def wgrads():
             dw = None
@@ -1522,16 +1641,21 @@
             return _unlayout_grads(dw, db, *ctx.wlayout)
 
         dw, db = wgrads()
-        return dx, dw, db, None, None, None, None, None, None
+        return dx, dw, db, None, None, None, None, None, None, None
 
 
 class PlainLinearFn(torch.autograd.Function):
 
     @staticmethod
-    def forward(ctx, x, weight, bias, splits: int, zero_bias_grad: bool, cdtype, col_index=None, n_cols=0, pad_rows=0):
+    def forward(ctx, x, weight, bias, splits: int, zero_bias_grad: bool, cdtype, col_index=None, n_cols=0, pad_rows=0, plain=None):
         L.require_gpu(x, weight)
         M, K = x.shape
-        w, bias_l = _layout_weight(weight, bias, cdtype, col_index, n_cols, pad_rows)
+        slot, packed = plain if plain is not None else (None, False)
+        if packed:
+            w, bf, wt = slot.W, slot.b, slot.Wt
+        else:
+            w, bias_l = _layout_weight(weight, bias, cdtype, col_index, n_cols, pad_rows)
+            bf, wt = (None if bias_l is None else bias_l.float().contiguous()), None
         N = w.shape[0]
         meta = LinearMeta(K=K, N=N, r_s=0, r_t=(), scale_s=0.0, scale_t=(), mode=0, has_x_tasks=False, dropout_p=0.0, seed=0,
                           dtype=cdtype)
@@ -1542,12 +1666,13 @@
             raise RuntimeError(f"mtlora_amd: invalid plain-linear shape M={M} K={K} N={N}")
         ctxbuf = torch.empty(max(ctx_bytes, 16), dtype=torch.uint8, device=x.device)
         y = torch.empty((M, N), dtype=cdtype, device=x.device)
-        bf = None if bias_l is None else bias_l.float().contiguous()
         st = lib.mtlora_linear_fwd(ctypes.byref(d), L.ptr(x), L.ptr_array(None), L.ptr(w), L.ptr(bf), L.ptr(None), L.ptr(None),
                                    L.ptr_array(None), L.ptr_array(None), L.ptr(y), L.ptr_array(None), L.ptr(ctxbuf), ctx_bytes,
                                    L.stream_ptr())
         L.check(st, "mtlora_linear_fwd (rank 0)")
         ctx.save_for_backward(x, w, ctxbuf)
+        ctx.wt = wt
+        ctx.plain, ctx.wcols = slot is not None, weight.shape[1]
         ctx.wlayout = (col_index, pad_rows)
         ctx.meta, ctx.splits, ctx.zero_bias_grad = meta, splits, zero_bias_grad
         ctx.has_bias, ctx.wdtype = bias is not None, weight.dtype
@@ -1567,12 +1692,16 @@
             lib = L.lib()
             sb = _desc_bytes("bwd", lib.mtlora_linear_bwd_scratch_bytes, ctx.meta, M, d)
             scratch = torch.empty(max(sb, 16), dtype=torch.uint8, device=x.device)
-            wt = w.t().contiguous()
+            wt = ctx.wt if ctx.wt is not None else w.t().contiguous()
             dx = torch.empty((M, K), dtype=x.dtype, device=x.device)
             st = lib.mtlora_linear_bwd(ctypes.byref(d), L.ptr(x), L.ptr_array(None), L.ptr(wt), L.ptr(gy), L.ptr_array(None),
                                        L.ptr(ctxbuf), ctxbuf.numel(), L.ptr(dx), L.ptr_array(None), L.ptr(None), L.ptr(None),
                                        L.ptr_array(None), L.ptr_array(None), L.ptr(scratch), sb, L.stream_ptr())
             L.check(st, "mtlora_linear_bwd (rank 0)")
+        if ctx.plain and ctx.needs_input_grad[1]:
+            dw, db = _plain_wgrads(ctx, gy, x, N, K, narrow_native=True)
+            return dx, dw, db, None, None, None, None, None, None, None
+
         def wgrads():
             dw = None
             if ctx.needs_input_grad[1]:
@@ -1590,7 +1719,7 @@
             return _unlayout_grads(dw, db, *ctx.wlayout)
 
         dw, db = wgrads()
-        return dx, dw, db, None, None, None, None, None, None
+        return dx, dw, db, None, None, None, None, None, None, None
 
 
 def gemm_tn(a: torch.Tensor, b: torch.Tensor) -> torch.Tensor:
@@ -1619,8 +1748,10 @@
     K, N = x.shape[1], weight.shape[0] + pad_rows
     if (_PLAIN_VIA_KNT and cdtype in _HOT_DTYPES and K % 8 == 0 and N % 8 == 0
             and x.dtype == cdtype):
-        return PlainLinearFn.apply(x, weight, bias, S, feeds_batchnorm, cdtype, col_index, K, pad_rows)
-    return SplitKLinearFn.apply(x, weight, bias, S, feeds_batchnorm, cdtype, col_index, K, pad_rows)
+        return PlainLinearFn.apply(x, weight, bias, S, feeds_batchnorm, cdtype, col_index, K, pad_rows,
+                                   _plain_lookup(weight, bias, cdtype, col_index, K, pad_rows))
+    return SplitKLinearFn.apply(x, weight, bias, S, feeds_batchnorm, cdtype, col_index, K, pad_rows,
+                                _plain_lookup(weight, bias, cdtype, col_index, K, pad_rows))
 
 
 def linear_big_m(x: torch.Tensor, weight: torch.Tensor, bias: Optional[torch.Tensor],
diff --git a/mtlora_amd/lora.py b/mtlora_amd/lora.py
--- a/mtlora_amd/lora.py
+++ b/mtlora_amd/lora.py
@@ -379,6 +379,43 @@
         return len(todo)
 
 
+class PlainPacker:
+
+    def __init__(self, model: nn.Module):
+        self.model = model
+        self._epoch = -1
+        self._params = []
+        self._table = None
+        self._table_key = None
+        self._tables = {}
+
+    def refresh(self) -> int:
+        if self._epoch != Fn._plain_epoch:
+            self._epoch = Fn._plain_epoch
+            self._params = [p for p in self.model.parameters() if getattr(p, "_mtlora_plain", None)]
+        todo = [(p, s) for p in self._params if p.is_cuda for s in p._mtlora_plain.values()]
+        if not todo:
+            return 0
+        key = tuple((id(s), p.data_ptr(), 0 if s.bias is None else s.bias.data_ptr()) for p, s in todo)
+        if key != self._table_key:
+            if key not in self._tables:
+                by_dtype = {}
+                for p, s in todo:
+                    if s.W is None:
+                        n, k = s.shape[0] + s.pad_rows, s.n_cols
+                        s.W = torch.empty((n, k), dtype=s.cdtype, device=p.device)
+                        s.Wt = torch.empty((k, n), dtype=s.cdtype, device=p.device)
+                        s.b = None if s.bias is None else torch.empty(n, dtype=torch.float32, device=p.device)
+                    by_dtype.setdefault((s.cdtype, str(p.device)), []).append((p, s))
+                self._tables[key] = [Fn.PlainPackTable(ents, ents[0][0].device, dt) for (dt, _), ents in by_dtype.items()]
+            self._table, self._table_key = self._tables[key], key
+        for tb in self._table:
+            tb.pack()
+        for p, s in todo:
+            s.stamp = s.current_stamp(p)
+        return len(todo)
+
+
 def mark_only_lora_as_trainable(model: nn.Module, bias: str = "none", freeze_patch_embed: bool = False,
                                 freeze_norm: bool = False, free_relative_bias: bool = False,
                                 freeze_downsample_reduction=False) -> None:
diff --git a/mtlora_amd/mtl_harness.py b/mtlora_amd/mtl_harness.py
--- a/mtlora_amd/mtl_harness.py
+++ b/mtlora_amd/mtl_harness.py
@@ -386,6 +386,15 @@
     return pk
 
 
+def _plain_packer(model):
+    pk = getattr(model, "_mtlora_plain_packer", None)
+    if pk is None:
+        from .lora import PlainPacker
+        pk = PlainPacker(model) if Fn._PLAIN_PACK else _NoPacker()
+        object.__setattr__(model, "_mtlora_plain_packer", pk)
+    return pk
+
+
 def train_step(model, criterion, optimizer, images, targets, clip_grad: float = 5.0, reducer=None,
                amp_dtype: Optional[torch.dtype] = torch.bfloat16, fused_loss: bool = True, loss_scaler=None,
                update_grad: bool = True):
@@ -403,6 +412,7 @@
     if images.is_cuda:
         Fn.droppath_begin_step(images.device)
         _factor_packer(model).refresh()
+        _plain_packer(model).refresh()
     try:
         if amp_dtype is not None:
             with torch.autocast("cuda", dtype=amp_dtype):
@@ -629,6 +639,7 @@
         self.seed.add_(self.SEED_STEP)
         if self.images.is_cuda:
             _factor_packer(self.model).refresh()
+            _plain_packer(self.model).refresh()
         ctx = (torch.autocast("cuda", dtype=self.amp_dtype, cache_enabled=False) if self.amp_dtype is not None
                else contextlib.nullcontext())
         with ctx:
```

Result: no change. 1149 images/sec (median of 6 runs) (+0.1%).
